# neeharperi/FutureDet

Measured on AMD Instinct MI355X. Metric: sweeps/sec end-to-end (300k pts, 10-sweep voxel), higher is better.
Workload: dtype f32

## Files before the change

### futuredet_amd/backbones.py

```python
import numpy as np
import torch
from torch import nn

from . import hip_ops, sparse as spconv
from .nn_utils import build_norm_layer
from .registry import BACKBONES
from .sparse import SparseConv3d, SubMConv3d


def conv3x3(in_planes, out_planes, stride=1, indice_key=None, bias=True):
    return spconv.SubMConv3d(in_planes, out_planes, kernel_size=3, stride=stride, padding=1, bias=bias,
                             indice_key=indice_key)


class SparseBasicBlock(spconv.SparseModule):
    expansion = 1

    def __init__(self, inplanes, planes, stride=1, norm_cfg=None, downsample=None, indice_key=None):
        super().__init__()
        if norm_cfg is None:
            norm_cfg = dict(type="BN1d", eps=1e-3, momentum=0.01)
        bias = norm_cfg is not None
        self.conv1 = conv3x3(inplanes, planes, stride, indice_key=indice_key, bias=bias)
        self.bn1 = build_norm_layer(norm_cfg, planes)[1]
        self.relu = nn.ReLU()
        self.conv2 = conv3x3(planes, planes, indice_key=indice_key, bias=bias)
        self.bn2 = build_norm_layer(norm_cfg, planes)[1]
        self.downsample = downsample
        self.stride = stride

    def forward(self, x):
        identity = x
        out = self.conv1(x)
        out.features = self.relu(self.bn1(out.features))
        out = self.conv2(out)
        out.features = self.bn2(out.features)
        if self.downsample is not None:
            identity = self.downsample(x)
        out.features = self.relu(out.features + identity.features)
        return out


@BACKBONES.register_module
class SpMiddleResNetFHD(nn.Module):
    def __init__(self, num_input_features=128, norm_cfg=None, name="SpMiddleResNetFHD", **kwargs):
        super().__init__()
        self.name = name
        if norm_cfg is None:
            norm_cfg = dict(type="BN1d", eps=1e-3, momentum=0.01)
        S = spconv.SparseSequential
        self.conv_input = S(SubMConv3d(num_input_features, 16, 3, bias=False, indice_key="res0"),
                            build_norm_layer(norm_cfg, 16)[1], nn.ReLU(inplace=True))
        self.conv1 = S(SparseBasicBlock(16, 16, norm_cfg=norm_cfg, indice_key="res0"),
                       SparseBasicBlock(16, 16, norm_cfg=norm_cfg, indice_key="res0"))
        self.conv2 = S(SparseConv3d(16, 32, 3, 2, padding=1, bias=False), build_norm_layer(norm_cfg, 32)[1],
                       nn.ReLU(inplace=True), SparseBasicBlock(32, 32, norm_cfg=norm_cfg, indice_key="res1"),
                       SparseBasicBlock(32, 32, norm_cfg=norm_cfg, indice_key="res1"))
        self.conv3 = S(SparseConv3d(32, 64, 3, 2, padding=1, bias=False), build_norm_layer(norm_cfg, 64)[1],
                       nn.ReLU(inplace=True), SparseBasicBlock(64, 64, norm_cfg=norm_cfg, indice_key="res2"),
                       SparseBasicBlock(64, 64, norm_cfg=norm_cfg, indice_key="res2"))
        self.conv4 = S(SparseConv3d(64, 128, 3, 2, padding=[0, 1, 1], bias=False), build_norm_layer(norm_cfg, 128)[1],
                       nn.ReLU(inplace=True), SparseBasicBlock(128, 128, norm_cfg=norm_cfg, indice_key="res3"),
                       SparseBasicBlock(128, 128, norm_cfg=norm_cfg, indice_key="res3"))
        self.extra_conv = S(SparseConv3d(128, 128, (3, 1, 1), (2, 1, 1), bias=False), build_norm_layer(norm_cfg, 128)[1],
                            nn.ReLU())
        self.compute_dtype = torch.float32
        self.dense_channels_last = True
        self.dense_dtype = None
        self.profile_hook = None

    def forward_generic(self, voxel_features, coors, batch_size, input_shape):
        sparse_shape = np.array(input_shape[::-1]) + [1, 0, 0]
        ret = spconv.SparseConvTensor(voxel_features, coors.int(), sparse_shape, batch_size)
        x = self.conv_input(ret)
        x_conv1 = self.conv1(x)
        x_conv2 = self.conv2(x_conv1)
        x_conv3 = self.conv3(x_conv2)
        x_conv4 = self.conv4(x_conv3)
        ret = self.extra_conv(x_conv4).dense()
        N, C, D, H, W = ret.shape
        ret = ret.view(N, C * D, H, W)
        return ret, {"conv1": x_conv1, "conv2": x_conv2, "conv3": x_conv3, "conv4": x_conv4}

    def _stages(self):
        return [(self.conv_input[0], self.conv_input[1], [self.conv1[0], self.conv1[1]], True),
                (self.conv2[0], self.conv2[1], [self.conv2[3], self.conv2[4]], False),
                (self.conv3[0], self.conv3[1], [self.conv3[3], self.conv3[4]], False),
                (self.conv4[0], self.conv4[1], [self.conv4[3], self.conv4[4]], False),
                (self.extra_conv[0], self.extra_conv[1], [], False)]

    def build_indexes(self, mark_fn, batch_size, input_shape, device, voxels=None, static=False, expected=None, row_caps=None):
        D, H, W = [int(v) for v in (np.array(input_shape[::-1]) + [1, 0, 0])]
        if voxels is not None:
            geoms = [self._stages()[lvl][0].geometry() for lvl in range(1, 5)]
            return hip_ops.build_pyramid(voxels[0], voxels[1], voxels[2], batch_size, (D, H, W), geoms, device, static=static,
                                         expected=expected, row_caps=row_caps)
        assert not static, "static indexes are built from the voxelizer's device output (voxels=...)"
        counts = torch.zeros((5,), dtype=torch.int32, device=device)
        idx = [hip_ops.SparseIndex(batch_size, D, H, W, device)]
        mark_fn(idx[0])
        idx[0].scan(counts[0:1])
        for lvl in range(1, 5):
            conv = self._stages()[lvl][0]
            ks, st, pd = conv.geometry()
            nxt = idx[-1].downsample(ks, st, pd)
            nxt.scan(counts[lvl:lvl + 1])
            idx.append(nxt)
        host = counts.cpu()
        for i, ix in enumerate(idx):
            ix.finalize(int(host[i]))
        return idx

    def run_fused(self, idx, feats0, dense_out=None, fork=False):
        dt = self.compute_dtype
        stages = self._stages()
        rb_cache = {}

        def rulebook(src, dst, conv):
            ks, st, pd = conv.geometry()
            key = (id(src), id(dst), tuple(ks), tuple(st), tuple(pd))
            if key not in rb_cache:
                rb_cache[key] = src.rulebook(dst, ks, st, pd)
            return rb_cache[key]

        def run(conv, bn, x, src, dst, relu, residual=None):
            wpk, bias, cin_p, cout_p = conv.packed_weight(dt, bn)
            assert x.shape[1] == cin_p, (x.shape, cin_p)
            nbr = rulebook(src, dst, conv)
            fn = lambda: hip_ops.spconv_apply(x, wpk, bias, nbr, dst.n, cout_p, residual=residual, relu=relu)
            if self.profile_hook is not None:
                s = 4 if dt == torch.float32 else 2
                K = nbr.shape[0]
                pairs = lambda: int((nbr[:, : dst.n] >= 0).sum().item())
                return self.profile_hook("spconv_%dx%d_K%d" % (cin_p, cout_p, K),
                                         dict(s=s, K=K, cin=cin_p, cout=cout_p, n_in=src.n, n_out=dst.n, pairs=pairs), fn)
            return fn()

        main, side = None, None
        if fork and feats0.is_cuda:
            main = torch.cuda.current_stream(feats0.device)
            pool = self.__dict__.setdefault("_side_streams", {})
            side = pool.get(main.cuda_stream)
            if side is None:
                side = pool[main.cuda_stream] = torch.cuda.Stream(device=feats0.device)
            side.wait_stream(main)
            with torch.cuda.stream(side):
                made = []
                for lvl, (conv, bn, blocks, is_subm_in) in enumerate(stages):
                    if lvl == 0:
                        continue
                    src_l, dst_l = (idx[lvl] if is_subm_in else idx[lvl - 1]), idx[lvl]
                    made.append(rulebook(src_l, dst_l, conv))
                    for blk in blocks:
                        nbr = rulebook(dst_l, dst_l, blk.conv1)
                        made.append(nbr)
                        cp = spconv.pad_channels(blk.conv1.out_channels)
                        if dt == torch.float32 and nbr.shape[0] == 27 and \
                                hip_ops._lib.load().fd_spconv_wants_balanced_ranges(cp, cp, 0):
                            r = hip_ops.ranges_for(nbr, cp, cp)
                            if r[0] is not None:
                                made.append(r[0])
                for t in made:
                    t.record_stream(main)
        x = feats0
        levels = {}
        for lvl, (conv, bn, blocks, is_subm_in) in enumerate(stages):
            src = idx[lvl] if is_subm_in else idx[lvl - 1]
            dst = idx[lvl]
            if lvl == 1 and side is not None:
                main.wait_stream(side)
            x = run(conv, bn, x, src, dst, relu=True)
            for blk in blocks:
                y = run(blk.conv1, blk.bn1, x, dst, dst, relu=True)
                x = run(blk.conv2, blk.bn2, y, dst, dst, relu=True, residual=x)
            levels[lvl] = (x, dst)
        bev = hip_ops.densify(x, idx[4], out_dtype=self.dense_dtype or dt, channels_last=self.dense_channels_last, out=dense_out)
        return bev, levels

    def forward(self, voxel_features, coors, batch_size, input_shape):
        if self.training:
            if self.compute_dtype != torch.float32 and torch.is_grad_enabled():
                raise NotImplementedError("SpMiddleResNetFHD: training runs the fp32 sparse convolution only; the %s path is inference-only "
                                          "(set compute_dtype = torch.float32 to train)" % self.compute_dtype)
            return self.forward_generic(voxel_features, coors, batch_size, input_shape)
        coors = coors.int().contiguous()
        dev = voxel_features.device
        idx = self.build_indexes(lambda i0: i0.mark(coors), batch_size, input_shape, dev)
        row_of = idx[0].lookup(coors)
        feats0 = hip_ops.rows_permute(voxel_features.float().contiguous(), row_of,
                                      spconv.pad_channels(voxel_features.shape[1]), self.compute_dtype, n_rows=idx[0].n)
        bev, levels = self.run_fused(idx, feats0)
        multi = {}
        for name, lvl, c in (("conv1", 0, 16), ("conv2", 1, 32), ("conv3", 2, 64), ("conv4", 3, 128)):
            f, ix = levels[lvl]
            multi[name] = spconv.SparseConvTensor(f[:, :c], None, ix.spatial_shape, batch_size, _index=ix)
        return bev, multi


@BACKBONES.register_module
class PointPillarsScatter(nn.Module):

    def __init__(self, num_input_features=64, norm_cfg=None, name="PointPillarsScatter", **kwargs):
        super().__init__()
        self.name = "PointPillarsScatter"
        self.nchannels = num_input_features
        self.dense_channels_last = True

    def forward(self, voxel_features, coords, batch_size, input_shape, n_dev=None):
        self.nx = int(input_shape[0])
        self.ny = int(input_shape[1])
        coords = coords.int().contiguous()
        if n_dev is None and torch.is_grad_enabled() and voxel_features.requires_grad:
            return _ScatterFn.apply(voxel_features, coords, batch_size, self.ny, self.nx, self.dense_channels_last)
        return hip_ops.pillar_scatter(voxel_features, coords, n_dev, batch_size, self.ny, self.nx,
                                      channels_last=self.dense_channels_last)


class _ScatterFn(torch.autograd.Function):

    @staticmethod
    def forward(ctx, feats, coords, batch_size, ny, nx, channels_last):
        ctx.coords = coords
        return hip_ops.pillar_scatter(feats, coords, None, batch_size, ny, nx, channels_last=channels_last)

    @staticmethod
    def backward(ctx, dcanvas):
        d = hip_ops.pillar_scatter_backward(dcanvas.float(), ctx.coords)
        ctx.coords = None
        return d, None, None, None, None, None
```

### futuredet_amd/csrc/fd_common.h

```cpp
#pragma once
#include <hip/hip_runtime.h>
#include <stdint.h>
#include <stdio.h>

#include <atomic>

#include "../../include/futuredet_hip.h"

namespace fd {

void set_error(const char *fmt, ...);
int spconv_f32_compact_dispatch(const float *in, const void *wp, const float *bias, const float *residual, int relu, const int *nbr,
                                int64_t nbr_stride, int K, int64_t n_in_bound, int n_out, const int *n_out_dev, int cin, int cout, float *out,
                                const int *ranges, int n_ranges, hipStream_t stream);

size_t spconv_bf16_win_weight_bytes(int K, int cin, int cout);
void spconv_bf16_win_pack(const float *w, int K, int cin, int cout, uint16_t (*tobf)(float), uint16_t *dst);
int spconv_bf16_win_dispatch(const void *in, const void *wp_win, const float *bias, const void *residual, int relu, const int *nbr, int64_t nbr_stride, int K,
                             int64_t n_in_bound, int n_out, const int *n_out_dev, int64_t n_expected, int cin, int cout, void *out, hipStream_t stream);
int spconv_bf16_ws_dispatch(const void *in, const void *wp, const float *bias, const void *residual, int relu, const int *nbr, int64_t nbr_stride, int K,
                            int64_t n_in_bound, int n_out, const int *n_out_dev, int64_t n_expected, int cin, int cout, void *out, hipStream_t stream);

int wino_pc_launch(const float *x, const void *wp, const float *bias, float *y, int B, int H, int W, int cin, int cout, int relu, int cout_total,
                   int co_off, int wide_items, hipStream_t stream);

int spconv_f32_res16_dispatch(const float *in, const void *wp, const float *bias, const float *residual, int relu, const int *nbr, int64_t nbr_stride, int K,
                              int64_t n_in_bound, int n_out, const int *n_out_dev, int64_t n_expected, int cin, int cout, float *out, hipStream_t stream);

int spconv_f32_c32_dispatch(const float *in, const void *wp, const float *bias, const float *residual, int relu, const int *nbr,
                            int64_t nbr_stride, int K, int64_t n_in_bound, int n_out, const int *n_out_dev, int cin, int cout, float *out,
                            const int *ranges, int n_ranges, hipStream_t stream);

__device__ __forceinline__ int device_count(int capacity, const int *count_dev) {
    if (!count_dev) return capacity;
    const int n = *count_dev;
    return n < capacity ? (n > 0 ? n : 0) : capacity;
}

inline int check_launch(const char *what) {
    hipError_t e = hipGetLastError();
    if (e != hipSuccess) {
        set_error("%s: %s", what, hipGetErrorString(e));
        return FD_ELAUNCH;
    }
    return FD_OK;
}

#define FD_REQUIRE(cond, ...)           \
    do {                                \
        if (!(cond)) {                  \
            fd::set_error(__VA_ARGS__); \
            return FD_EINVAL;           \
        }                               \
    } while (0)

inline hipStream_t as_stream(fd_stream_t s) { return reinterpret_cast<hipStream_t>(s); }

int fill_words(void *p, uint32_t value, size_t n_words, hipStream_t stream);
int fill_words3(void *p0, uint32_t v0, size_t n0, void *p1, uint32_t v1, size_t n1, void *p2, uint32_t v2, size_t n2, hipStream_t stream);

constexpr int kMaxDevices = 64;
int current_device();
int device_cu_count();
bool ensure_dynamic_lds(const void *kernel, size_t bytes, std::atomic<uint64_t> &done);
enum TuneKey { kTuneSpconvRG = 0, kTuneSpconvV1, kTuneSpconvBf16V1, kTuneV2Depth, kTuneV2TM, kTuneV2LdsPad, kTuneConvNT, kTuneV2RangesPerCU, kTuneV2Uniform, kTuneV2RowCost, kTuneSpconvC32, kTuneBf16GP, kTuneBf16RG, kTuneBf16Depth, kTuneBf16NW, kTuneStrict, kTuneBf16Win, kTuneF32ResRG, kTuneConvStrip, kTuneF32ResNW, kTuneCount };
int tuning(TuneKey key);

inline size_t align_up(size_t v, size_t a) { return (v + a - 1) / a * a; }

struct IndexGeom {
    int B, D, H, W, Ht, Wt;
    __host__ __device__ int64_t num_cols() const { return (int64_t)B * Ht * Wt * 64; }
};
__host__ __device__ inline IndexGeom make_geom(int B, int D, int H, int W) {
    IndexGeom g;
    g.B = B; g.D = D; g.H = H; g.W = W;
    g.Ht = (H + 7) >> 3; g.Wt = (W + 7) >> 3;
    return g;
}
__host__ __device__ inline int64_t col_of(const IndexGeom &g, int b, int y, int x) {
    return ((((int64_t)b * g.Ht + (y >> 3)) * g.Wt + (x >> 3)) << 6) + ((y & 7) << 3) + (x & 7);
}
__device__ inline void col_to_byx(const IndexGeom &g, int64_t col, int &b, int &y, int &x) {
    int in = (int)(col & 63);
    int64_t t = col >> 6;
    int tx = (int)(t % g.Wt);
    t /= g.Wt;
    int ty = (int)(t % g.Ht);
    b = (int)(t / g.Ht);
    y = ty * 8 + (in >> 3);
    x = tx * 8 + (in & 7);
}

__device__ inline unsigned xcd_swizzle(unsigned bid, unsigned nblocks) {
    const unsigned nx = 8;
    unsigned per = nblocks / nx, rem = nblocks % nx;
    unsigned xcd = bid % nx, loc = bid / nx;
    unsigned start = xcd * per + (xcd < rem ? xcd : rem);
    return start + loc;
}

}
```

### futuredet_amd/csrc/fd_spconv.hip

```cpp
#include "fd_common.h"

namespace {

typedef float f32x4 __attribute__((ext_vector_type(4)));
typedef short s16x4 __attribute__((ext_vector_type(4)));
typedef __bf16 bf16x8 __attribute__((ext_vector_type(8)));

__device__ inline unsigned short f2bf(float v) {
    unsigned u = __float_as_uint(v);
    u += 0x7fffu + ((u >> 16) & 1u);
    return (unsigned short)(u >> 16);
}
__device__ inline float bf2f(unsigned short h) { return __uint_as_float(((unsigned)h) << 16); }

constexpr int kMaxTaps = 27;

template <int CIN, int COUT, int RG>
__global__ void __launch_bounds__(256) spconv_f32(const float *__restrict__ in, const float4 *__restrict__ wp,
                                                  const float *__restrict__ bias, const float *__restrict__ residual, int relu,
                                                  const int *__restrict__ nbr, int64_t nbr_stride, int K, int n_out,
                                                  const int *__restrict__ n_out_dev, float *__restrict__ out) {
    constexpr int ROWS_B = 64 * RG;
    constexpr int NB = COUT / 16, NC = CIN / 16;
    __shared__ int s_nbr[kMaxTaps * ROWS_B];
    const int tile = blockIdx.x;
    const int row0 = tile * ROWS_B;
    n_out = fd::device_count(n_out, n_out_dev);
    if (row0 >= n_out) return;
    for (int t = threadIdx.x; t < K * ROWS_B; t += 256) {
        int k = t / ROWS_B, r = t - k * ROWS_B;
        int64_t o = (int64_t)row0 + r;
        s_nbr[t] = (o < n_out) ? nbr[(int64_t)k * nbr_stride + o] : -1;
    }
    __syncthreads();
    const int lane = threadIdx.x & 63, wave = __builtin_amdgcn_readfirstlane(threadIdx.x >> 6);
    const int lrow = lane & 15, lq = lane >> 4;
    const int wrow = wave * 16 * RG;
    if (row0 + wrow >= n_out) return;

    f32x4 acc[RG][NB];
#pragma unroll
    for (int g = 0; g < RG; ++g)
#pragma unroll
        for (int nb = 0; nb < NB; ++nb) acc[g][nb] = (f32x4){0.f, 0.f, 0.f, 0.f};

    for (int k = 0; k < K; ++k) {
        int idx[RG];
        bool any[RG];
        bool any_all = false;
#pragma unroll
        for (int g = 0; g < RG; ++g) {
            idx[g] = s_nbr[k * ROWS_B + wrow + g * 16 + lrow];
            any[g] = __ballot(idx[g] >= 0) != 0ull;
            any_all = any_all || any[g];
        }
        if (!any_all) continue;
        const float4 *wk = wp + (int64_t)k * NC * NB * 64 + lane;
#pragma unroll
        for (int c = 0; c < NC; ++c) {
            float4 a[RG];
#pragma unroll
            for (int g = 0; g < RG; ++g) {
                a[g] = make_float4(0.f, 0.f, 0.f, 0.f);
                if (idx[g] >= 0) a[g] = *reinterpret_cast<const float4 *>(in + (int64_t)idx[g] * CIN + c * 16 + lq * 4);
            }
#pragma unroll
            for (int nb = 0; nb < NB; ++nb) {
                const float4 b = wk[(c * NB + nb) * 64];
#pragma unroll
                for (int g = 0; g < RG; ++g) {
                    if (any[g]) {
                        acc[g][nb] = __builtin_amdgcn_mfma_f32_16x16x4f32(a[g].x, b.x, acc[g][nb], 0, 0, 0);
                        acc[g][nb] = __builtin_amdgcn_mfma_f32_16x16x4f32(a[g].y, b.y, acc[g][nb], 0, 0, 0);
                        acc[g][nb] = __builtin_amdgcn_mfma_f32_16x16x4f32(a[g].z, b.z, acc[g][nb], 0, 0, 0);
                        acc[g][nb] = __builtin_amdgcn_mfma_f32_16x16x4f32(a[g].w, b.w, acc[g][nb], 0, 0, 0);
                    }
                }
            }
        }
    }
#pragma unroll
    for (int g = 0; g < RG; ++g) {
#pragma unroll
        for (int nb = 0; nb < NB; ++nb) {
            const int col = nb * 16 + lrow;
            const float bv = bias ? bias[col] : 0.0f;
#pragma unroll
            for (int r = 0; r < 4; ++r) {
                const int row = row0 + wrow + g * 16 + lq * 4 + r;
                if (row < n_out) {
                    float v = acc[g][nb][r] + bv;
                    if (residual) v += residual[(int64_t)row * COUT + col];
                    if (relu) v = fmaxf(v, 0.0f);
                    out[(int64_t)row * COUT + col] = v;
                }
            }
        }
    }
}

template <int CIN, int COUT, int RG>
__global__ void __launch_bounds__(256) spconv_bf16(const unsigned short *__restrict__ in, const void *__restrict__ wp_,
                                                   const float *__restrict__ bias, const unsigned short *__restrict__ residual,
                                                   int relu, const int *__restrict__ nbr, int64_t nbr_stride, int K, int n_out,
                                                   const int *__restrict__ n_out_dev, unsigned short *__restrict__ out) {
    constexpr int ROWS_B = 64 * RG;
    constexpr int NB = COUT / 16;
    constexpr bool WIDE = CIN >= 32;
    constexpr int NC = WIDE ? CIN / 32 : 1;
    __shared__ int s_nbr[kMaxTaps * ROWS_B];
    const int tile = blockIdx.x;
    const int row0 = tile * ROWS_B;
    n_out = fd::device_count(n_out, n_out_dev);
    if (row0 >= n_out) return;
    for (int t = threadIdx.x; t < K * ROWS_B; t += 256) {
        int k = t / ROWS_B, r = t - k * ROWS_B;
        int64_t o = (int64_t)row0 + r;
        s_nbr[t] = (o < n_out) ? nbr[(int64_t)k * nbr_stride + o] : -1;
    }
    __syncthreads();
    const int lane = threadIdx.x & 63, wave = __builtin_amdgcn_readfirstlane(threadIdx.x >> 6);
    const int lrow = lane & 15, lq = lane >> 4;
    const int wrow = wave * 16 * RG;
    if (row0 + wrow >= n_out) return;

    f32x4 acc[RG][NB];
#pragma unroll
    for (int g = 0; g < RG; ++g)
#pragma unroll
        for (int nb = 0; nb < NB; ++nb) acc[g][nb] = (f32x4){0.f, 0.f, 0.f, 0.f};

    for (int k = 0; k < K; ++k) {
        int idx[RG];
        bool any[RG];
        bool any_all = false;
#pragma unroll
        for (int g = 0; g < RG; ++g) {
            idx[g] = s_nbr[k * ROWS_B + wrow + g * 16 + lrow];
            any[g] = __ballot(idx[g] >= 0) != 0ull;
            any_all = any_all || any[g];
        }
        if (!any_all) continue;
        if constexpr (WIDE) {
            const bf16x8 *wk = reinterpret_cast<const bf16x8 *>(wp_) + (int64_t)k * NC * NB * 64 + lane;
#pragma unroll
            for (int c = 0; c < NC; ++c) {
                bf16x8 a[RG];
#pragma unroll
                for (int g = 0; g < RG; ++g) {
                    uint4 raw = make_uint4(0u, 0u, 0u, 0u);
                    if (idx[g] >= 0) raw = *reinterpret_cast<const uint4 *>(in + (int64_t)idx[g] * CIN + c * 32 + lq * 8);
                    a[g] = __builtin_bit_cast(bf16x8, raw);
                }
#pragma unroll
                for (int nb = 0; nb < NB; ++nb) {
                    const bf16x8 b = wk[(c * NB + nb) * 64];
#pragma unroll
                    for (int g = 0; g < RG; ++g)
                        if (any[g]) acc[g][nb] = __builtin_amdgcn_mfma_f32_16x16x32_bf16(a[g], b, acc[g][nb], 0, 0, 0);
                }
            }
        } else {
            const s16x4 *wk = reinterpret_cast<const s16x4 *>(wp_) + (int64_t)k * NB * 64 + lane;
            s16x4 a[RG];
#pragma unroll
            for (int g = 0; g < RG; ++g) {
                uint2 raw = make_uint2(0u, 0u);
                if (idx[g] >= 0) raw = *reinterpret_cast<const uint2 *>(in + (int64_t)idx[g] * CIN + lq * 4);
                a[g] = __builtin_bit_cast(s16x4, raw);
            }
#pragma unroll
            for (int nb = 0; nb < NB; ++nb) {
                const s16x4 b = wk[nb * 64];
#pragma unroll
                for (int g = 0; g < RG; ++g)
                    if (any[g]) acc[g][nb] = __builtin_amdgcn_mfma_f32_16x16x16bf16_1k(a[g], b, acc[g][nb], 0, 0, 0);
            }
        }
    }
#pragma unroll
    for (int g = 0; g < RG; ++g) {
#pragma unroll
        for (int nb = 0; nb < NB; ++nb) {
            const int col = nb * 16 + lrow;
            const float bv = bias ? bias[col] : 0.0f;
#pragma unroll
            for (int r = 0; r < 4; ++r) {
                const int row = row0 + wrow + g * 16 + lq * 4 + r;
                if (row < n_out) {
                    float v = acc[g][nb][r] + bv;
                    if (residual) v += bf2f(residual[(int64_t)row * COUT + col]);
                    if (relu) v = fmaxf(v, 0.0f);
                    out[(int64_t)row * COUT + col] = f2bf(v);
                }
            }
        }
    }
}

struct LaunchArgs {
    const void *in, *wp;
    const float *bias;
    const void *residual;
    int relu;
    const int *nbr;
    int64_t nbr_stride;
    int K, n_out;
    const int *n_out_dev;
    void *out;
    hipStream_t stream;
};

template <int CIN, int COUT, int RG>
void launch(const LaunchArgs &a, int dtype) {
    const int rows_b = 64 * RG;
    dim3 grid((unsigned)((a.n_out + rows_b - 1) / rows_b));
    if (dtype == 0)
        hipLaunchKernelGGL((spconv_f32<CIN, COUT, RG>), grid, dim3(256), 0, a.stream, (const float *)a.in, (const float4 *)a.wp, a.bias,
                           (const float *)a.residual, a.relu, a.nbr, a.nbr_stride, a.K, a.n_out, a.n_out_dev, (float *)a.out);
    else
        hipLaunchKernelGGL((spconv_bf16<CIN, COUT, RG>), grid, dim3(256), 0, a.stream, (const unsigned short *)a.in, a.wp, a.bias,
                           (const unsigned short *)a.residual, a.relu, a.nbr, a.nbr_stride, a.K, a.n_out, a.n_out_dev, (unsigned short *)a.out);
}

template <int CIN, int COUT>
void launch_rg(const LaunchArgs &a, int dtype, int rg) {
    if (rg >= 4) launch<CIN, COUT, 4>(a, dtype);
    else if (rg == 2) launch<CIN, COUT, 2>(a, dtype);
    else launch<CIN, COUT, 1>(a, dtype);
}

int pick_rg(int64_t n_out, int cin, int cout) {
    const int forced = fd::tuning(fd::kTuneSpconvRG);
    if (forced > 0) return forced;
    const int64_t waves2 = (n_out + 31) / 32;
    int rg = (cin * cout >= 128 * 128) ? 1 : 2;
    if (rg == 2 && waves2 < 256 * 4 * 2) rg = 1;
    return rg;
}

}

inline bool has_c32_layout(int cin, int cout, int dtype) { return dtype == 0 && cout == 32 && cin == 32; }
inline int64_t pair_layout_elems(int K, int cin, int cout, int dtype) { return (dtype == 1 && cin == 16) ? (int64_t)((K + 1) / 2) * 32 * cout : 0; }

extern "C" size_t fd_spconv_packed_weight_bytes(int K, int cin, int cout, int dtype) {
    if (K <= 0 || cin <= 0 || cout <= 0) return 0;
    return (size_t)K * cin * cout * (dtype == 0 ? 4 : 2) * (has_c32_layout(cin, cout, dtype) ? 2 : 1) + (size_t)pair_layout_elems(K, cin, cout, dtype) * 2 +
           (dtype == 1 ? fd::spconv_bf16_win_weight_bytes(K, cin, cout) : 0);
}

extern "C" int fd_spconv_pack_weight(const float *w, int K, int cin, int cout, int dtype, void *dst) {
    FD_REQUIRE(w && dst, "fd_spconv_pack_weight: null argument");
    FD_REQUIRE(K >= 1 && K <= kMaxTaps, "fd_spconv_pack_weight: K must be in [1,27]");
    FD_REQUIRE(cin % 16 == 0 && cout % 16 == 0 && cin >= 16 && cin <= 128 && cout >= 16 && cout <= 128,
               "fd_spconv_pack_weight: channels must be multiples of 16 in [16,128] (got %d -> %d)", cin, cout);
    FD_REQUIRE(dtype == 0 || dtype == 1, "fd_spconv_pack_weight: dtype must be 0 (f32) or 1 (bf16)");
    const int NB = cout / 16;
    auto W = [&](int k, int ci, int co) { return w[((int64_t)k * cin + ci) * cout + co]; };
    auto tobf = [](float v) -> uint16_t {
        union { float f; uint32_t u; } cvt;
        cvt.f = v;
        uint32_t u = cvt.u;
        u += 0x7fffu + ((u >> 16) & 1u);
        return (uint16_t)(u >> 16);
    };
    if (dtype == 0) {
        const int NC = cin / 16;
        float *d = (float *)dst;
        for (int k = 0; k < K; ++k)
            for (int c = 0; c < NC; ++c)
                for (int nb = 0; nb < NB; ++nb)
                    for (int lane = 0; lane < 64; ++lane)
                        for (int j = 0; j < 4; ++j)
                            d[((((int64_t)k * NC + c) * NB + nb) * 64 + lane) * 4 + j] =
                                W(k, 16 * c + 4 * (lane >> 4) + j, 16 * nb + (lane & 15));
        if (has_c32_layout(cin, cout, dtype)) {
            float *e = d + (int64_t)K * cin * cout;
            for (int k = 0; k < K; ++k)
                for (int c = 0; c < cin / 8; ++c)
                    for (int lane = 0; lane < 64; ++lane)
                        for (int j = 0; j < 4; ++j)
                            e[(((int64_t)k * (cin / 8) + c) * 64 + lane) * 4 + j] = W(k, 8 * c + 4 * (lane >> 5) + j, lane & 31);
        }
    } else if (cin >= 32) {
        FD_REQUIRE(cin % 32 == 0, "fd_spconv_pack_weight: bf16 needs cin 16 or a multiple of 32");
        const int NC = cin / 32;
        uint16_t *d = (uint16_t *)dst;
        for (int k = 0; k < K; ++k)
            for (int c = 0; c < NC; ++c)
                for (int nb = 0; nb < NB; ++nb)
                    for (int lane = 0; lane < 64; ++lane)
                        for (int j = 0; j < 8; ++j)
                            d[((((int64_t)k * NC + c) * NB + nb) * 64 + lane) * 8 + j] =
                                tobf(W(k, 32 * c + 8 * (lane >> 4) + j, 16 * nb + (lane & 15)));
        if (fd::spconv_bf16_win_weight_bytes(K, cin, cout)) fd::spconv_bf16_win_pack(w, K, cin, cout, +tobf, d + (int64_t)K * cin * cout);
    } else {
        uint16_t *d = (uint16_t *)dst;
        for (int k = 0; k < K; ++k)
            for (int nb = 0; nb < NB; ++nb)
                for (int lane = 0; lane < 64; ++lane)
                    for (int j = 0; j < 4; ++j)
                        d[(((int64_t)k * NB + nb) * 64 + lane) * 4 + j] = tobf(W(k, 4 * (lane >> 4) + j, 16 * nb + (lane & 15)));
        uint16_t *e = d + (int64_t)K * cin * cout;
        for (int u = 0; u < (K + 1) / 2; ++u)
            for (int nb = 0; nb < NB; ++nb)
                for (int lane = 0; lane < 64; ++lane)
                    for (int j = 0; j < 8; ++j) {
                        const int q = lane >> 4, k = 2 * u + (q >> 1);
                        e[(((int64_t)u * NB + nb) * 64 + lane) * 8 + j] = k < K ? tobf(W(k, 8 * (q & 1) + j, 16 * nb + (lane & 15))) : (uint16_t)0;
                    }
    }
    return FD_OK;
}

extern "C" int fd_spconv_apply(const void *in_feats, int64_t n_in, const void *wpacked, const float *bias, const void *residual, int relu,
                               const int32_t *nbr, int64_t nbr_stride, const int32_t *ranges, int n_ranges, int K, int64_t n_out,
                               const int32_t *n_out_dev, int64_t n_expected, int cin, int cout, int dtype, void *out_feats, fd_stream_t stream) {
    FD_REQUIRE(K >= 1 && K <= kMaxTaps, "fd_spconv_apply: K must be in [1,27]");
    FD_REQUIRE(dtype == 0 || dtype == 1, "fd_spconv_apply: dtype must be 0 (f32) or 1 (bf16)");
    FD_REQUIRE(n_out >= 0 && n_out <= nbr_stride && n_out < (1ll << 31), "fd_spconv_apply: n_out out of range");
    FD_REQUIRE(n_ranges >= 0 && (ranges == nullptr || n_ranges >= 1), "fd_spconv_apply: ranges needs n_ranges >= 1");
    if (n_expected <= 0 || n_expected > n_out) n_expected = n_out;
    if (n_out == 0) return FD_OK;
    FD_REQUIRE(in_feats && wpacked && nbr && out_feats, "fd_spconv_apply: null argument");
    if (dtype == 0 && !fd::tuning(fd::kTuneSpconvV1) && cin == 16 && fd::tuning(fd::kTuneF32ResRG) >= 0) {
        if (fd::spconv_f32_res16_dispatch((const float *)in_feats, wpacked, bias, (const float *)residual, relu, nbr, nbr_stride, K, n_in, (int)n_out,
                                          n_out_dev, n_expected, cin, cout, (float *)out_feats, fd::as_stream(stream)))
            return fd::check_launch("fd_spconv_apply(f32 resident)");
    }
    if (dtype == 0 && !fd::tuning(fd::kTuneSpconvV1) && has_c32_layout(cin, cout, dtype) && fd::tuning(fd::kTuneSpconvC32) >= 0) {
        const void *w32 = (const char *)wpacked + (size_t)K * cin * cout * 4;
        if (fd::spconv_f32_c32_dispatch((const float *)in_feats, w32, bias, (const float *)residual, relu, nbr, nbr_stride, K, n_in, (int)n_out,
                                        n_out_dev, cin, cout, (float *)out_feats, ranges, n_ranges, fd::as_stream(stream)))
            return fd::check_launch("fd_spconv_apply(c32)");
    }
    if (dtype == 0 && !fd::tuning(fd::kTuneSpconvV1)) {
        if (fd::spconv_f32_compact_dispatch((const float *)in_feats, wpacked, bias, (const float *)residual, relu, nbr, nbr_stride, K, n_in,
                                            (int)n_out, n_out_dev, cin, cout, (float *)out_feats, ranges, n_ranges, fd::as_stream(stream)))
            return fd::check_launch("fd_spconv_apply(compact)");
    }
    if (dtype == 1 && fd::tuning(fd::kTuneBf16GP) >= 0) {
        const void *w = cin == 16 ? (const void *)((const char *)wpacked + (size_t)K * cin * cout * 2) : wpacked;
        const bool subm_like = (K == 27 && n_in == n_out) || fd::tuning(fd::kTuneBf16Win) == 2;
        if (fd::tuning(fd::kTuneBf16Win) >= 0 && subm_like && fd::spconv_bf16_win_weight_bytes(K, cin, cout) &&
            fd::spconv_bf16_win_dispatch(in_feats, (const char *)wpacked + (size_t)K * cin * cout * 2, bias, residual, relu, nbr, nbr_stride, K, n_in, (int)n_out,
                                         n_out_dev, n_expected, cin, cout, out_feats, fd::as_stream(stream)))
            return fd::check_launch("fd_spconv_apply(bf16 window)");
        if (fd::spconv_bf16_ws_dispatch(in_feats, w, bias, residual, relu, nbr, nbr_stride, K, n_in, (int)n_out, n_out_dev, n_expected, cin, cout, out_feats,
                                        fd::as_stream(stream)))
            return fd::check_launch("fd_spconv_apply(bf16 ws)");
        if (fd::tuning(fd::kTuneStrict) && n_in * cin * 2 < (1ll << 31)) {
            fd::set_error("fd_spconv_apply: strict mode: the bf16 kernel (fd_spconv_bf16.hip) did not take %d -> %d, K = %d", cin, cout, K);
            return FD_EINVAL;
        }
    }
    LaunchArgs a{in_feats, wpacked, bias, residual, relu, nbr, nbr_stride, K, (int)n_out, n_out_dev, out_feats, fd::as_stream(stream)};
    const int rg = pick_rg(n_expected, cin, cout);
    const int key = cin * 1000 + cout;
    switch (key) {
        case 16016: launch_rg<16, 16>(a, dtype, rg); break;
        case 16032: launch_rg<16, 32>(a, dtype, rg); break;
        case 32032: launch_rg<32, 32>(a, dtype, rg); break;
        case 32064: launch_rg<32, 64>(a, dtype, rg); break;
        case 64064: launch_rg<64, 64>(a, dtype, rg); break;
        case 64128: launch_rg<64, 128>(a, dtype, rg); break;
        case 128128: launch_rg<128, 128>(a, dtype, rg); break;
        default:
            fd::set_error("fd_spconv_apply: unsupported channels %d -> %d", cin, cout);
            return FD_EINVAL;
    }
    return fd::check_launch("fd_spconv_apply");
}
```

### futuredet_amd/csrc/fd_spconv_c32.hip

```cpp
#include "fd_spconv_chunk.h"

namespace {

namespace sk = fd::skeleton;
typedef float f32x16 __attribute__((ext_vector_type(16)));
typedef unsigned u32x4 __attribute__((ext_vector_type(4)));
constexpr int TM = 128, COUT = 32, TS = 4, WR = 1;
constexpr sk::Layout L = sk::layout(TM, COUT, TS, 32);
static_assert(((sk::kMaxTaps + TS - 1) / TS) * (TM / WR / 32) <= L.item_slot, "item list slot");

template <int CIN, int DEPTH>
__global__ void __launch_bounds__(256) spconv_f32_c32(const float *__restrict__ in, const float4 *__restrict__ wp, const float *__restrict__ bias,
                                                      const float *__restrict__ residual, int relu, const int *__restrict__ nbr, int64_t nbr_stride,
                                                      int K, int n_out, const int *__restrict__ n_out_dev, float *__restrict__ out, unsigned in_bytes,
                                                      const int *__restrict__ ranges, int rows_per_range) {
    constexpr int NCH = CIN / 8;
    constexpr int kPad = sk::pad_entry(TM);
    extern __shared__ __attribute__((aligned(16))) unsigned char smem[];
    int *s_list = reinterpret_cast<int *>(smem + L.list);
    unsigned short *s_items = reinterpret_cast<unsigned short *>(smem + L.items);
    unsigned char *s_cnt = smem + L.cnt;
    int *s_pad = reinterpret_cast<int *>(smem + L.pad);
    float *s_acc = reinterpret_cast<float *>(smem + L.acc);

    const int tid = threadIdx.x, lane = tid & 63, wave = __builtin_amdgcn_readfirstlane(tid >> 6);
    int r_begin, r_end, n_chunks, chunk_rows;
    sk::resolve_range(n_out, n_out_dev, ranges, rows_per_range, r_begin, r_end);
    if (r_begin >= r_end) return;
    sk::cut_chunks<TM>(r_begin, r_end, n_chunks, chunk_rows);
    int pre[sk::kSliceRegs<TM>];
    sk::fetch_slice<TM>(pre, nbr, nbr_stride, K, r_begin);

    const int ln = lane & 31, lh = lane >> 5;
    const int ts = wave, wr = 0;
    unsigned char *acc_bytes = reinterpret_cast<unsigned char *>(s_acc + ts * L.acc_copy);
    const __amdgpu_buffer_rsrc_t rsrc = __builtin_amdgcn_make_buffer_rsrc(const_cast<float *>(in), 0, (int)in_bytes, 0x00020000);
    unsigned short *items = s_items + wave * L.item_slot;

    for (int chunk = 0; chunk < n_chunks; ++chunk) {
        int row0, n_rows;
        if (!sk::chunk_span(r_begin, r_end, chunk_rows, chunk, row0, n_rows)) break;
        sk::stage_chunk<TM, COUT, TS, 32>(pre, s_list, s_pad, s_acc, bias, residual, K, row0, n_rows);
        __syncthreads();
        sk::compact_taps<TM, WR>(s_list, s_cnt, K);
        __syncthreads();
        if (chunk + 1 < n_chunks) sk::fetch_slice<TM>(pre, nbr, nbr_stride, K, row0 + chunk_rows);
        const int n_items = sk::build_items<TS, 32>(s_cnt, items, K, ts, wr);

        int k_r[DEPTH], row_r[DEPTH];
        u32x4 a_r[DEPTH][NCH];
        auto stage_a0 = [&](int it) -> int { return sk::stage_a0(items, n_items, it); };
        auto stage_a1 = [&](int it, int code_v, int &kk, int &e) { sk::stage_a1<TM, WR, 32>(s_list, s_pad, n_items, wr, ln, it, code_v, kk, e); };
        auto gather_offset = [&](int e) -> unsigned { return sk::entry_row_bytes<CIN>(e) + (unsigned)(lh * 16); };
        auto gather_step = [&](unsigned voff, int c) { return __builtin_amdgcn_raw_buffer_load_b128(rsrc, voff + c * 32, 0, 0); };
        float4 b[NCH];
        auto load_b = [&](int k) {
            const float4 *wk = wp + (int64_t)k * NCH * 64 + lane;
#pragma unroll
            for (int c = 0; c < NCH; ++c) b[c] = wk[c * 64];
        };
        int k_s, e_s, code_s;
#pragma unroll
        for (int d = 0; d < DEPTH - 1; ++d) {
            stage_a1(d, stage_a0(d), k_s, e_s);
            const unsigned vo = gather_offset(e_s);
#pragma unroll
            for (int c = 0; c < NCH; ++c) a_r[d][c] = gather_step(vo, c);
            k_r[d] = k_s;
            row_r[d] = e_s;
        }
        k_r[DEPTH - 1] = -1;
        row_r[DEPTH - 1] = kPad;
        stage_a1(DEPTH - 1, stage_a0(DEPTH - 1), k_s, e_s);
        code_s = stage_a0(DEPTH);
        if (n_items > 0) load_b(k_r[0]);

        for (int i0 = 0; i0 < n_items; i0 += DEPTH) {
#pragma unroll
            for (int d = 0; d < DEPTH; ++d) {
                const unsigned arow = sk::entry_local_row(row_r[d]);
                unsigned aoff[4];
#pragma unroll
                for (int q = 0; q < 4; ++q) aoff[q] = sk::acc_slot_bytes<COUT>(arow, (unsigned)(2 * q + lh));
                f32x16 acc;
#pragma unroll
                for (int q = 0; q < 4; ++q) {
                    const float4 v = *reinterpret_cast<const float4 *>(acc_bytes + aoff[q]);
                    acc[4 * q + 0] = v.x; acc[4 * q + 1] = v.y; acc[4 * q + 2] = v.z; acc[4 * q + 3] = v.w;
                }
                const int dn = (d + DEPTH - 1) % DEPTH;
                {
                    const int it = i0 + d + DEPTH - 1;
                    const unsigned vo = gather_offset(e_s);
                    k_r[dn] = k_s;
                    row_r[dn] = e_s;
#pragma unroll
                    for (int c = 0; c < NCH; ++c) a_r[dn][c] = gather_step(vo, c);
                    stage_a1(it + 1, code_s, k_s, e_s);
                    code_s = stage_a0(it + 2);
                }
                const int knext = k_r[(d + 1) % DEPTH];
                const bool reload = knext >= 0 && knext != k_r[d];
                __builtin_amdgcn_sched_barrier(0);
#pragma unroll
                for (int c = 0; c < NCH; ++c) {
                    const float4 av = __builtin_bit_cast(float4, a_r[d][c]);
                    acc = __builtin_amdgcn_mfma_f32_32x32x2f32(b[c].x, av.x, acc, 0, 0, 0);
                    acc = __builtin_amdgcn_mfma_f32_32x32x2f32(b[c].y, av.y, acc, 0, 0, 0);
                    acc = __builtin_amdgcn_mfma_f32_32x32x2f32(b[c].z, av.z, acc, 0, 0, 0);
                    acc = __builtin_amdgcn_mfma_f32_32x32x2f32(b[c].w, av.w, acc, 0, 0, 0);
                    if (reload) b[c] = (wp + (int64_t)knext * NCH * 64 + lane)[c * 64];
                }
#pragma unroll
                for (int q = 0; q < 4; ++q)
                    *reinterpret_cast<float4 *>(acc_bytes + aoff[q]) = make_float4(acc[4 * q + 0], acc[4 * q + 1], acc[4 * q + 2], acc[4 * q + 3]);
                __builtin_amdgcn_sched_barrier(0);
            }
        }
        __syncthreads();
        sk::epilogue<TM, COUT, TS>(s_acc, bias, residual, relu, out, row0, n_rows);
        __syncthreads();
    }
}

template <int CIN, int DEPTH>
int launch_c32(const float *in, const void *wp, const float *bias, const float *residual, int relu, const int *nbr, int64_t nbr_stride, int K,
               int n_out, const int *n_out_dev, float *out, unsigned in_bytes, const int *ranges, int n_ranges, hipStream_t stream) {
    int rows_per = 0;
    if (!ranges) sk::equal_rows_split(n_out, TM, n_out_dev != nullptr, n_ranges, rows_per);
    static std::atomic<uint64_t> lds_set{0};
    if (!fd::ensure_dynamic_lds(reinterpret_cast<const void *>(spconv_f32_c32<CIN, DEPTH>), (size_t)L.bytes, lds_set)) return 0;
    hipLaunchKernelGGL((spconv_f32_c32<CIN, DEPTH>), dim3((unsigned)n_ranges), dim3(256), (size_t)L.bytes, stream, in, (const float4 *)wp, bias, residual, relu,
                       nbr, nbr_stride, K, n_out, n_out_dev, out, in_bytes, ranges, rows_per);
    return 1;
}

}

namespace fd {
int spconv_f32_c32_dispatch(const float *in, const void *wp, const float *bias, const float *residual, int relu, const int *nbr, int64_t nbr_stride,
                            int K, int64_t n_in_bound, int n_out, const int *n_out_dev, int cin, int cout, float *out, const int *ranges,
                            int n_ranges, hipStream_t stream) {
    if (cout != 32 || cin != 32) return 0;
    if (!sk::entries_fit(n_in_bound, cin)) return 0;
    const unsigned in_bytes = (unsigned)(n_in_bound * cin * 4);
    const int depth = fd::tuning(fd::kTuneV2Depth);
    if (depth == 2) return launch_c32<32, 2>(in, wp, bias, residual, relu, nbr, nbr_stride, K, n_out, n_out_dev, out, in_bytes, ranges, n_ranges, stream);
    if (depth == 4) return launch_c32<32, 4>(in, wp, bias, residual, relu, nbr, nbr_stride, K, n_out, n_out_dev, out, in_bytes, ranges, n_ranges, stream);
    return launch_c32<32, 3>(in, wp, bias, residual, relu, nbr, nbr_stride, K, n_out, n_out_dev, out, in_bytes, ranges, n_ranges, stream);
}
}
```

### futuredet_amd/csrc/fd_spconv_chunk.h

```cpp
#pragma once
#include "fd_common.h"

namespace fd {
namespace skeleton {

constexpr int kMaxTaps = 27;

constexpr int pad_entry(int tm) { return (int)(0xffffff00u | (unsigned)tm); }
__device__ __forceinline__ int pack_entry(int in_row, int local_row) { return (in_row << 8) | local_row; }
__device__ __forceinline__ unsigned entry_local_row(int e) { return (unsigned)e & 255u; }
template <int CIN>
__device__ __forceinline__ unsigned entry_row_bytes(int e) {
    static_assert(CIN == 16 || CIN == 32 || CIN == 64 || CIN == 128, "shift per CIN");
    const unsigned hi = (unsigned)e & 0xffffff00u;
    return CIN >= 64 ? hi << (CIN == 128 ? 1 : 0) : hi >> (CIN == 32 ? 1 : 2);
}
inline bool entries_fit(int64_t n_in_bound, int cin) { return n_in_bound < (1ll << 23) && n_in_bound * cin * 4 < (1ll << 31); }

struct Layout {
    int list;
    int items;
    int item_slot;
    int cnt;
    int pad;
    int acc;
    int acc_copy;
    int bytes;
};
constexpr int acc_copy_floats(int tm, int cout) { return (tm + 1) * cout; }
constexpr Layout layout(int tm, int cout, int ts, int item) {
    Layout l{};
    l.list = 0;
    l.items = l.list + (int)sizeof(int) * kMaxTaps * tm;
    l.item_slot = item == 16 ? kMaxTaps * (tm / 16) : 32;
    l.cnt = l.items + (int)sizeof(unsigned short) * 4 * l.item_slot;
    l.pad = l.cnt + 112;
    l.acc = l.pad + (int)sizeof(int) * item;
    l.acc_copy = acc_copy_floats(tm, cout);
    l.bytes = l.acc + (int)sizeof(float) * ts * l.acc_copy;
    return l;
}

template <int COUT>
__device__ __forceinline__ unsigned acc_swizzle(unsigned row) {
    static_assert(COUT == 16 || COUT == 32 || COUT == 64 || COUT == 128, "whole bank rows");
    constexpr int kSwzShift = COUT >= 64 ? 0 : COUT == 32 ? 1 : 2;
    constexpr unsigned kSwzMask = COUT >= 64 ? 15u : COUT == 32 ? 7u : 3u;
    return (row >> kSwzShift) & kSwzMask;
}
template <int COUT>
__device__ __forceinline__ int acc_slot(int row, int col) {
    return row * (COUT / 4) + (col ^ (int)acc_swizzle<COUT>((unsigned)row));
}
template <int COUT>
__device__ __forceinline__ unsigned acc_slot_bytes(unsigned row, unsigned col) {
    return row * (COUT * 4) + ((col ^ acc_swizzle<COUT>(row)) << 4);
}

__device__ __forceinline__ void resolve_range(int n_out, const int *n_out_dev, const int *ranges, int rows_per_range,
                                              int &r_begin, int &r_end) {
    if (n_out_dev) n_out = fd::device_count(n_out, n_out_dev);
    if (ranges) {
        r_begin = ranges[blockIdx.x];
        r_end = ranges[blockIdx.x + 1];
    } else {
        if (n_out_dev) rows_per_range = (((n_out + (int)gridDim.x - 1) / (int)gridDim.x) + 15) & ~15;
        const int64_t b = (int64_t)blockIdx.x * rows_per_range;
        r_begin = (int)(b < n_out ? b : n_out);
        r_end = (int)(b + rows_per_range < n_out ? b + rows_per_range : n_out);
    }
    if (r_end > n_out) r_end = n_out;
}
template <int TM>
__device__ __forceinline__ void cut_chunks(int r_begin, int r_end, int &n_chunks, int &chunk_rows) {
    n_chunks = (r_end - r_begin + TM - 1) / TM;
    chunk_rows = (((r_end - r_begin + n_chunks - 1) / n_chunks) + 15) & ~15;
}
__device__ __forceinline__ bool chunk_span(int r_begin, int r_end, int chunk_rows, int chunk, int &row0, int &n_rows) {
    row0 = r_begin + chunk * chunk_rows;
    n_rows = (r_end - row0) < chunk_rows ? (r_end - row0) : chunk_rows;
    return n_rows > 0;
}
inline void equal_rows_split(int n_out, int tm, bool device_count, int &n_ranges, int &rows_per) {
    if (n_ranges <= 0) n_ranges = (n_out + tm - 1) / tm;
    rows_per = (((n_out + n_ranges - 1) / n_ranges) + 15) & ~15;
    if (!device_count) n_ranges = (n_out + rows_per - 1) / rows_per;
}

template <int TM>
constexpr int kSliceRegs = (kMaxTaps * TM + 255) / 256;

template <int TM>
__device__ __forceinline__ void fetch_slice(int (&pre)[kSliceRegs<TM>], const int *nbr, int64_t nbr_stride, int K, int row0) {
    const int tid = threadIdx.x;
#pragma unroll
    for (int i = 0; i < kSliceRegs<TM>; ++i) {
        const int t = tid + i * 256;
        int k = t / TM;
        const int r = t - k * TM;
        k = k < K ? k : K - 1;
        int64_t o = (int64_t)row0 + r;
        o = o < nbr_stride ? o : nbr_stride - 1;
        pre[i] = nbr[(int64_t)k * nbr_stride + o];
    }
}

template <int COUT>
constexpr bool kInitAcc = COUT <= 64;

template <int TM, int COUT, int TS>
__device__ __forceinline__ void init_acc(float *s_acc, const float *bias, const float *residual, int row0, int n_rows) {
    const int tid = threadIdx.x;
    if constexpr (kInitAcc<COUT>) {
        constexpr int C4i = COUT / 4, NINIT = TM * C4i / 256;
        static_assert(TM * C4i % 256 == 0, "whole passes");
        float4 iv[NINIT];
#pragma unroll
        for (int i = 0; i < NINIT; ++i) {
            const int t = tid + i * 256, c4 = t % C4i;
            iv[i] = bias ? reinterpret_cast<const float4 *>(bias)[c4] : make_float4(0.f, 0.f, 0.f, 0.f);
        }
        if (residual) {
            float4 rv[NINIT];
#pragma unroll
            for (int i = 0; i < NINIT; ++i) {
                const int t = tid + i * 256, r = t / C4i, c4 = t - r * C4i;
                const int rr = r < n_rows ? r : n_rows - 1;
                rv[i] = reinterpret_cast<const float4 *>(residual + (int64_t)(row0 + rr) * COUT)[c4];
            }
#pragma unroll
            for (int i = 0; i < NINIT; ++i) { iv[i].x += rv[i].x; iv[i].y += rv[i].y; iv[i].z += rv[i].z; iv[i].w += rv[i].w; }
        }
#pragma unroll
        for (int i = 0; i < NINIT; ++i) {
            const int t = tid + i * 256, r = t / C4i, c4 = t - r * C4i;
            reinterpret_cast<float4 *>(s_acc)[acc_slot<COUT>(r, c4)] = r < n_rows ? iv[i] : make_float4(0.f, 0.f, 0.f, 0.f);
        }
        for (int t = TM * C4i + tid; t < TS * acc_copy_floats(TM, COUT) / 4; t += 256) reinterpret_cast<float4 *>(s_acc)[t] = make_float4(0.f, 0.f, 0.f, 0.f);
    } else {
        for (int t = tid; t < TS * acc_copy_floats(TM, COUT) / 4; t += 256) reinterpret_cast<float4 *>(s_acc)[t] = make_float4(0.f, 0.f, 0.f, 0.f);
    }
}

template <int TM, int COUT, int TS, int ITEM>
__device__ __forceinline__ void stage_chunk(const int (&pre)[kSliceRegs<TM>], int *s_list, int *s_pad, float *s_acc, const float *bias,
                                            const float *residual, int K, int row0, int n_rows) {
    const int tid = threadIdx.x;
    static_assert(256 % TM == 0, "a thread stages the same local row in every pass");
    const bool in_chunk = tid % TM < n_rows;
#pragma unroll
    for (int i = 0; i < kSliceRegs<TM>; ++i) {
        const int t = tid + i * 256;
        if (t < K * TM) s_list[t] = in_chunk ? pre[i] : -1;
    }
    init_acc<TM, COUT, TS>(s_acc, bias, residual, row0, n_rows);
    if (tid < ITEM) s_pad[tid] = pad_entry(TM);
}

template <int TM, int WR>
__device__ __forceinline__ void compact_taps(int *s_list, unsigned char *s_cnt, int K) {
    const int lane = threadIdx.x & 63, wave = __builtin_amdgcn_readfirstlane(threadIdx.x >> 6);
    constexpr int RW = TM / WR, NH = (RW + 63) / 64;
    for (int k = wave; k < K; k += 4) {
#pragma unroll
        for (int wr = 0; wr < WR; ++wr) {
            const int base = k * TM + wr * RW;
            int count = 0;
            int v[NH];
#pragma unroll
            for (int h = 0; h < NH; ++h) {
                const int r = h * 64 + lane;
                v[h] = (r < RW) ? s_list[base + r] : -1;
            }
#pragma unroll
            for (int h = 0; h < NH; ++h) {
                const int r = h * 64 + lane;
                if (r < RW) s_list[base + r] = pad_entry(TM);
            }
#pragma unroll
            for (int h = 0; h < NH; ++h) {
                const int r = h * 64 + lane;
                const unsigned long long m = __ballot(v[h] >= 0);
                const int pos = count + __popcll(m & ((1ull << lane) - 1ull));
                if (v[h] >= 0) s_list[base + pos] = pack_entry(v[h], wr * RW + r);
                count += __popcll(m);
            }
            if (lane == 0) s_cnt[k * 4 + wr] = (unsigned char)count;
        }
    }
}

template <int TS, int ITEM>
__device__ __forceinline__ int build_items(const unsigned char *s_cnt, unsigned short *items, int K, int ts, int wr) {
    const int lane = threadIdx.x & 63;
    const int ng = (lane < K && (lane % TS) == ts) ? ((int)s_cnt[lane * 4 + wr] + ITEM - 1) / ITEM : 0;
    int inc = ng;
#pragma unroll
    for (int off = 1; off < 64; off <<= 1) {
        const int u = __shfl_up(inc, off);
        if (lane >= off) inc += u;
    }
    const int n_items = __builtin_amdgcn_readfirstlane(__shfl(inc, 63));
    for (int g = 0; g < ng; ++g) items[inc - ng + g] = (unsigned short)((lane << 3) | g);
    __builtin_amdgcn_fence(__ATOMIC_RELEASE, "workgroup");
    __builtin_amdgcn_wave_barrier();
    __builtin_amdgcn_fence(__ATOMIC_ACQUIRE, "workgroup");
    return n_items;
}

__device__ __forceinline__ int stage_a0(const unsigned short *items, int n_items, int it) { return (int)items[it < n_items ? it : 0]; }
template <int TM, int WR, int ITEM>
__device__ __forceinline__ void stage_a1(const int *s_list, const int *s_pad, int n_items, int wr, int lp, int it, int code_v, int &kk, int &e) {
    const bool v = it < n_items;
    const int code = __builtin_amdgcn_readfirstlane(code_v);
    const int ks = v ? (code >> 3) : 0;
    kk = v ? ks : -1;
    const int *lst = v ? s_list + ks * TM + wr * (TM / WR) + (code & 7) * ITEM : s_pad;
    e = lst[lp];
}

template <int TM, int COUT, int TS>
__device__ __forceinline__ void epilogue(float *s_acc, const float *bias, const float *residual, int relu,
                                         float *out, int row0, int n_rows) {
    const int tid = threadIdx.x;
    constexpr int C4 = COUT / 4;
    for (int t = tid; t < n_rows * C4; t += 256) {
        const int r = t / C4, c4 = t - r * C4;
        const int row = row0 + r;
        const int slot = acc_slot<COUT>(r, c4);
        float4 v = reinterpret_cast<const float4 *>(s_acc)[slot];
#pragma unroll
        for (int q = 1; q < TS; ++q) {
            const float4 v2 = reinterpret_cast<const float4 *>(s_acc + q * acc_copy_floats(TM, COUT))[slot];
            v.x += v2.x; v.y += v2.y; v.z += v2.z; v.w += v2.w;
        }
        if constexpr (!kInitAcc<COUT>) {
            if (bias) {
                const float4 bv = reinterpret_cast<const float4 *>(bias)[c4];
                v.x += bv.x; v.y += bv.y; v.z += bv.z; v.w += bv.w;
            }
            if (residual) {
                const float4 rv = reinterpret_cast<const float4 *>(residual + (int64_t)row * COUT)[c4];
                v.x += rv.x; v.y += rv.y; v.z += rv.z; v.w += rv.w;
            }
        }
        if (relu) { v.x = fmaxf(v.x, 0.f); v.y = fmaxf(v.y, 0.f); v.z = fmaxf(v.z, 0.f); v.w = fmaxf(v.w, 0.f); }
        reinterpret_cast<float4 *>(out + (int64_t)row * COUT)[c4] = v;
    }
}

}
}
```

### futuredet_amd/hip_ops.py

```python
import ctypes
import threading

import numpy as np
import torch

from . import lib as _lib
from .lib import DecodeCfg, FutureDetHipError, MapView, check


_raw_stream = getattr(torch._C, "_cuda_getCurrentRawStream", None)


def _stream():
    if _raw_stream is not None:
        return ctypes.c_void_p(_raw_stream(torch.cuda.current_device()))
    return ctypes.c_void_p(torch.cuda.current_stream().cuda_stream)


def _dev(t, name, dtype=None):
    if not isinstance(t, torch.Tensor) or not t.is_cuda:
        raise FutureDetHipError("%s must be a tensor on the HIP device (got %s); this path has no CPU implementation"
                                % (name, "cpu tensor" if isinstance(t, torch.Tensor) else type(t)))
    if dtype is not None and t.dtype != dtype:
        raise FutureDetHipError("%s must be %s, got %s" % (name, dtype, t.dtype))
    if not t.is_contiguous():
        raise FutureDetHipError("%s must be contiguous" % name)
    return t


def _p(t):
    return ctypes.c_void_p(t.data_ptr()) if t is not None else None


class _Workspace(object):

    def __init__(self):
        self._bufs = {}
        self._scope = threading.local()

    def scope(self, token):
        ws = self

        class _Scope(object):
            def __enter__(self_):
                self_.prev = getattr(ws._scope, "token", None)
                ws._scope.token = token

            def __exit__(self_, *exc):
                ws._scope.token = self_.prev

        return _Scope()

    def release(self, token):
        for key in [k for k in self._bufs if k[2] == ("scope", token)]:
            del self._bufs[key]

    def get(self, tag, nbytes, device):
        token = getattr(self._scope, "token", None)
        key = (tag, device.index, ("scope", token) if token is not None else _stream().value)
        buf = self._bufs.get(key)
        if buf is None or buf.numel() < nbytes:
            buf = torch.empty(max(int(nbytes), 256), dtype=torch.uint8, device=device)
            self._bufs[key] = buf
        return buf


workspace = _Workspace()
_DT = {torch.float32: 0, torch.bfloat16: 1}


def set_tuning(name, value):
    check(_lib.load().fd_tuning_set(name.encode(), int(value)), "fd_tuning_set")


def voxelize(points, voxel_size, coors_range, max_points, max_voxels, batch_idx=0, want_voxels=True, want_mean=False,
             mean_stride=None, coor_cols=3, out=None, n_points_dev=None):
    L = _lib.load()
    points = _dev(points, "points", torch.float32)
    n, ndim = points.shape
    dev = points.device
    rng = (ctypes.c_float * 6)(*[float(np.float32(v)) for v in coors_range])
    vs = (ctypes.c_float * 3)(*[float(np.float32(v)) for v in voxel_size])
    out = dict(out or {})
    if want_voxels and "voxels" not in out:
        out["voxels"] = torch.empty((max_voxels, max_points, ndim), dtype=torch.float32, device=dev)
    if want_mean and "mean" not in out:
        out["mean"] = torch.empty((max_voxels, mean_stride or ndim), dtype=torch.float32, device=dev)
    if "coors" not in out:
        out["coors"] = torch.empty((max_voxels, coor_cols), dtype=torch.int32, device=dev)
    if "num_points" not in out:
        out["num_points"] = torch.empty((max_voxels,), dtype=torch.int32, device=dev)
    if "num_voxels" not in out:
        out["num_voxels"] = torch.zeros((1,), dtype=torch.int32, device=dev)
    mean = out.get("mean") if want_mean else None
    voxels = out.get("voxels") if want_voxels else None
    ws_bytes = L.fd_voxelize_workspace_bytes(n, max_voxels)
    ws = workspace.get("voxelize", ws_bytes, dev)
    check(L.fd_voxelize(_p(points), n, _p(n_points_dev), ndim, rng, vs, int(max_points), int(max_voxels), int(batch_idx), _p(voxels), _p(mean),
                        int(mean.shape[1]) if mean is not None else 0, _p(out["coors"]), int(out["coors"].shape[1]),
                        _p(out["num_points"]), _p(out["num_voxels"]), _p(ws), ws.numel(), _stream()), "fd_voxelize")
    return out


class SparseIndex(object):

    def __init__(self, B, D, H, W, device, words=None, prefix=None):
        L = _lib.load()
        self.B, self.D, self.H, self.W = int(B), int(D), int(H), int(W)
        self.ncols = L.fd_index_num_cols(self.B, self.H, self.W)
        self.words = torch.zeros((self.ncols,), dtype=torch.int64, device=device) if words is None else words
        self.prefix = torch.empty((self.ncols,), dtype=torch.int32, device=device) if prefix is None else prefix
        self.n_dev = None
        self.n = None
        self.coords = None
        self.device = device
        self.static = False
        self.n_expected = 0

    @property
    def spatial_shape(self):
        return [self.D, self.H, self.W]

    def mark(self, coords, n_dev=None, n_max=None):
        L = _lib.load()
        coords = _dev(coords, "coords", torch.int32)
        n_max = coords.shape[0] if n_max is None else n_max
        check(L.fd_index_mark(_p(coords), _p(n_dev), n_max, self.B, self.D, self.H, self.W, _p(self.words), _stream()),
              "fd_index_mark")

    def scan(self, n_dev):
        L = _lib.load()
        ws = workspace.get("index_scan", L.fd_index_workspace_bytes(self.ncols), self.device)
        self.n_dev = n_dev
        check(L.fd_index_scan(_p(self.words), self.ncols, _p(self.prefix), _p(n_dev), _p(ws), ws.numel(), _stream()),
              "fd_index_scan")

    def downsample(self, ksize, stride, pad):
        L = _lib.load()
        od = [(i + 2 * p - (k - 1) - 1) // s + 1 for i, k, s, p in zip(self.spatial_shape, ksize, stride, pad)]
        out = SparseIndex(self.B, od[0], od[1], od[2], self.device)
        check(L.fd_index_downsample(_p(self.words), self.B, self.D, self.H, self.W, (ctypes.c_int * 3)(*ksize),
                                    (ctypes.c_int * 3)(*stride), (ctypes.c_int * 3)(*pad), _p(out.words), _stream()),
              "fd_index_downsample")
        return out

    def finalize(self, n):
        L = _lib.load()
        self.n = int(n)
        self.coords = torch.empty((max(self.n, 1), 4), dtype=torch.int32, device=self.device)[: self.n]
        if self.n:
            check(L.fd_index_coords(_p(self.words), _p(self.prefix), self.B, self.D, self.H, self.W, _p(self.coords),
                                    _stream()), "fd_index_coords")

    def lookup(self, coords, n_dev=None):
        L = _lib.load()
        coords = _dev(coords, "coords", torch.int32)
        row_of = torch.empty((coords.shape[0],), dtype=torch.int32, device=self.device)
        check(L.fd_index_lookup(_p(self.words), _p(self.prefix), self.B, self.D, self.H, self.W, _p(coords), _p(n_dev),
                                coords.shape[0], _p(row_of), _stream()), "fd_index_lookup")
        return row_of

    def rulebook(self, out_index, ksize, stride, pad):
        L = _lib.load()
        assert out_index.n is not None
        K = int(ksize[0] * ksize[1] * ksize[2])
        nstride = max(64, (out_index.n + 63) // 64 * 64)
        nbr = torch.empty((K, nstride), dtype=torch.int32, device=self.device)
        static = getattr(out_index, "static", False)
        if out_index.n == 0:
            nbr.fill_(-1)
            return nbr
        check(L.fd_rulebook(_p(self.words), _p(self.prefix), self.B, self.D, self.H, self.W, _p(out_index.coords), out_index.n,
                            _p(out_index.n_dev), nstride, 0 if static else 1, (ctypes.c_int * 3)(*ksize), (ctypes.c_int * 3)(*stride),
                            (ctypes.c_int * 3)(*pad), _p(nbr), _stream()), "fd_rulebook")
        nbr.n_out = out_index.n
        nbr.n_dev = out_index.n_dev if static else None
        nbr.n_expected = out_index.n_expected if static else 0
        return nbr


class _PyramidPlan(object):

    def __init__(self, B, shape0, geoms, device):
        L = _lib.load()
        self.B, self.geoms, self.device = int(B), geoms, device
        self.shapes = [tuple(int(v) for v in shape0)]
        for ks, st, pd in geoms:
            self.shapes.append(tuple((i + 2 * p - (k - 1) - 1) // s + 1 for i, k, s, p in zip(self.shapes[-1], ks, st, pd)))
        self.ncols = [L.fd_index_num_cols(self.B, sh[1], sh[2]) for sh in self.shapes]
        self.ws_bytes = L.fd_index_workspace_bytes(sum(self.ncols) + 2048 * len(self.ncols))

    def row_caps(self, cap0):
        caps = [min(int(cap0), self.B * int(np.prod(self.shapes[0])))]
        for (ks, st, pd), sh in zip(self.geoms, self.shapes[1:]):
            fan = int(np.prod([-(-k // s) for k, s in zip(ks, st)]))
            caps.append(min(caps[-1] * fan, self.B * int(np.prod(sh))))
        return caps


_pyramid_plans = {}


def build_pyramid(coors, nvox, n_max, B, shape0, geoms, device, static=False, expected=None, row_caps=None):
    L = _lib.load()
    key = (int(B), tuple(int(v) for v in shape0), tuple((tuple(k), tuple(s), tuple(p)) for k, s, p in geoms), str(device))
    plan = _pyramid_plans.get(key)
    if plan is None:
        plan = _pyramid_plans[key] = _PyramidPlan(B, shape0, geoms, device)
    shapes, ncols = plan.shapes, plan.ncols
    words_all = torch.empty((sum(ncols),), dtype=torch.int64, device=device)
    prefix_all = torch.empty((sum(ncols),), dtype=torch.int32, device=device)
    counts = torch.empty((len(shapes),), dtype=torch.int32, device=device)
    idx, off = [], 0
    levels = (_lib.IndexLevel * len(shapes))()
    wp, pp = words_all.data_ptr(), prefix_all.data_ptr()
    for l, (sh, nc) in enumerate(zip(shapes, ncols)):
        ix = SparseIndex.__new__(SparseIndex)
        ix.B, ix.D, ix.H, ix.W, ix.ncols, ix.device = plan.B, sh[0], sh[1], sh[2], nc, device
        ix.words, ix.prefix = words_all[off:off + nc], prefix_all[off:off + nc]
        ix.n_dev, ix.n, ix.coords = counts[l:l + 1], None, None
        ix.level_counts = counts
        ix.static, ix.n_expected = False, 0
        lv = levels[l]
        lv.D, lv.H, lv.W = sh
        if l:
            ks, st, pd = geoms[l - 1]
            lv.ksize[:], lv.stride[:], lv.pad[:] = list(ks), list(st), list(pd)
        lv.words, lv.prefix, lv.coords = wp + 8 * off, pp + 4 * off, None
        idx.append(ix)
        off += nc
    ws = workspace.get("index_scan", plan.ws_bytes, device)

    def size_coords(host):
        total = sum(host)
        coords_all = torch.empty((max(total, 1), 4), dtype=torch.int32, device=device)
        o = 0
        for l, ix in enumerate(idx):
            ix.n = int(host[l])
            ix.coords = coords_all[o:o + ix.n]
            levels[l].coords = (coords_all.data_ptr() + 16 * o) if ix.n else None
            levels[l].coords_rows = ix.n
            o += ix.n

    if static:
        host = plan.row_caps(int(B) * int(n_max))
        if row_caps is not None:
            host = [min(int(a), int(b)) for a, b in zip(host, row_caps)]
        for l, ix in enumerate(idx):
            ix.static = True
            ix.n_expected = int(expected[l]) if expected is not None else 0
        size_coords(host)
        fused = all(int(h) > 0 for h in host)
        check(L.fd_index_pyramid(_p(coors), _p(nvox), int(n_max), plan.B, len(shapes), levels, _p(counts), _p(ws), ws.numel(), _stream()),
              "fd_index_pyramid")
        if not fused:
            check(L.fd_index_pyramid_coords(plan.B, len(shapes), levels, _stream()), "fd_index_pyramid_coords")
        return idx
    check(L.fd_index_pyramid(_p(coors), _p(nvox), int(n_max), plan.B, len(shapes), levels, _p(counts), _p(ws), ws.numel(), _stream()),
          "fd_index_pyramid")
    size_coords(counts.tolist())
    check(L.fd_index_pyramid_coords(plan.B, len(shapes), levels, _stream()), "fd_index_pyramid_coords")
    return idx


def ranges_for(nbr, cin, cout):
    cached = getattr(nbr, "ranges", None)
    if cached is not None:
        return cached
    L = _lib.load()
    n_out = getattr(nbr, "n_out", None)
    if not n_out:
        return None, 0
    K, nstride = nbr.shape
    n = int(L.fd_spconv_num_ranges(getattr(nbr, "n_expected", 0) or n_out, cin, cout, 0))
    if n <= 0:
        return None, 0
    ranges = torch.empty((n + 1,), dtype=torch.int32, device=nbr.device)
    ws = workspace.get("spconv_ranges", L.fd_spconv_ranges_workspace_bytes(n_out), nbr.device)
    check(L.fd_spconv_ranges(_p(nbr), nstride, K, n_out, _p(getattr(nbr, "n_dev", None)), n, _p(ranges), _p(ws), ws.numel(), _stream()),
          "fd_spconv_ranges")
    nbr.ranges = (ranges, n)
    return nbr.ranges


def rows_permute(src, row_of, c_dst, dtype=torch.float32, n_rows=None, n_dev=None):
    L = _lib.load()
    src = _dev(src, "src", torch.float32)
    row_of = _dev(row_of, "row_of", torch.int32)
    n_rows = src.shape[0] if n_rows is None else n_rows
    dst = torch.zeros((max(n_rows, 1), c_dst), dtype=dtype, device=src.device)[:n_rows]
    if src.shape[0]:
        check(L.fd_rows_permute(_p(src), src.shape[1], _p(row_of), _p(n_dev), src.shape[0], _p(dst), c_dst,
                                _DT[dtype], _stream()), "fd_rows_permute")
    return dst


def rows_place(index, coords, src, c_dst, dtype=torch.float32, n_dev=None, out=None):
    L = _lib.load()
    coords = _dev(coords, "coords", torch.int32)
    src = _dev(src, "src", torch.float32)
    if out is None:
        out = torch.zeros((max(index.n, 1), c_dst), dtype=dtype, device=src.device)[: index.n]
    _dev(out, "out", dtype)
    if coords.dim() != 2 or coords.shape[1] != 4:
        raise FutureDetHipError("rows_place: coords must be [n, 4] (b, z, y, x), got %s" % (tuple(coords.shape),))
    if src.dim() != 2 or src.shape[0] < coords.shape[0]:
        raise FutureDetHipError("rows_place: src must be [n, c_src] with a row per coordinate")
    if out.dim() != 2 or out.shape[1] != c_dst or index.n is None or out.shape[0] < index.n:
        raise FutureDetHipError("rows_place: out must be [rows >= index.n, %d] (finalised index), got %s" % (c_dst, tuple(out.shape)))
    check(L.fd_rows_place(_p(index.words), _p(index.prefix), index.B, index.D, index.H, index.W, _p(coords), _p(n_dev),
                          coords.shape[0], _p(src), src.shape[1], _p(out), c_dst, _DT[dtype], _stream()), "fd_rows_place")
    return out


def pack_spconv_weight(w_kio, dtype=torch.float32):
    L = _lib.load()
    dev = w_kio.device
    w = w_kio.detach().to("cpu", torch.float32).contiguous()
    K, cin, cout = w.shape
    nbytes = L.fd_spconv_packed_weight_bytes(K, cin, cout, _DT[dtype])
    host = torch.empty((nbytes,), dtype=torch.uint8)
    check(L.fd_spconv_pack_weight(ctypes.c_void_p(w.data_ptr()), K, cin, cout, _DT[dtype], ctypes.c_void_p(host.data_ptr())),
          "fd_spconv_pack_weight")
    return host.to(dev)


PACK_PLAIN, PACK_TRANSPOSED, PACK_FLIPPED_TRANSPOSED = 0, 1, 2


def pack_spconv_weight_device(w_kio, mode=PACK_PLAIN):
    L = _lib.load()
    w = _dev(w_kio.detach(), "w_kio", torch.float32)
    K, cin, cout = w.shape
    ci, co = (cout, cin) if mode else (cin, cout)
    out = torch.empty((L.fd_spconv_packed_weight_bytes(K, ci, co, 0),), dtype=torch.uint8, device=w.device)
    check(L.fd_spconv_pack_weight_device(_p(w), K, cin, cout, int(mode), _p(out), _stream()), "fd_spconv_pack_weight_device")
    return out


def spconv_wgrad(feats, dy, nbr, n_out):
    L = _lib.load()
    feats = _dev(feats, "feats", torch.float32)
    dy = _dev(dy, "dy", torch.float32)
    K, nstride = nbr.shape
    cin, cout = feats.shape[1], dy.shape[1]
    assert dy.shape[0] >= n_out
    dw = torch.empty((K, cin, cout), dtype=torch.float32, device=feats.device)
    ws = workspace.get("spconv_wgrad", L.fd_spconv_wgrad_workspace_bytes(K, n_out, cin, cout), feats.device)
    check(L.fd_spconv_wgrad(_p(feats), feats.shape[0], _p(dy), _p(_dev(nbr, "nbr", torch.int32)), nstride, K, n_out,
                            _p(getattr(nbr, "n_dev", None)), cin, cout, _p(dw), _p(ws), ws.numel(), _stream()), "fd_spconv_wgrad")
    return dw


def assign_targets(boxes, counts, classes, trajectory, cfg, out):
    L = _lib.load()
    boxes = _dev(boxes, "boxes", torch.float32)
    B = boxes.shape[0]
    assert tuple(boxes.shape) == (B, cfg.T, cfg.n_max, 12), (tuple(boxes.shape), cfg.T, cfg.n_max)
    assert tuple(counts.shape) == (B, cfg.T) and tuple(classes.shape) == (B, cfg.T, cfg.n_max)
    assert (trajectory is None) == (cfg.n_sets == 1)
    if trajectory is not None:
        assert tuple(trajectory.shape) == (B, cfg.T, cfg.n_max)
        trajectory = _dev(trajectory, "trajectory", torch.int32)
    U = cfg.n_tasks + (2 if cfg.n_sets == 3 else 0)
    ws = workspace.get("targets", L.fd_targets_workspace_bytes(B, cfg.T, U, cfg.max_objs), boxes.device)
    check(L.fd_assign_targets(_p(boxes), _p(_dev(counts, "counts", torch.int32)), _p(_dev(classes, "classes", torch.int32)), _p(trajectory), B,
                              ctypes.byref(cfg), _p(_dev(out["hm"], "hm", torch.float32)), _p(_dev(out["ind"], "ind", torch.int64)),
                              _p(_dev(out["mask"], "mask", torch.uint8)), _p(_dev(out["cat"], "cat", torch.int64)),
                              _p(_dev(out["anno_box"], "anno_box", torch.float32)), _p(_dev(out["gt_boxes_and_cls"], "gt_boxes_and_cls", torch.float32)),
                              _p(_dev(out["status"], "status", torch.int32)), _p(ws), ws.numel(), _stream()), "fd_assign_targets")
    return out


def rulebook_transpose(nbr, n_out, n_in):
    L = _lib.load()
    K, nstride = nbr.shape
    istride = max(64, (n_in + 63) // 64 * 64)
    inv = torch.empty((K, istride), dtype=torch.int32, device=nbr.device)
    check(L.fd_rulebook_transpose(_p(_dev(nbr, "nbr", torch.int32)), nstride, K, n_out, _p(getattr(nbr, "n_dev", None)), n_in, _p(inv),
                                  istride, _stream()), "fd_rulebook_transpose")
    return inv


def dense_gather(grad, index, c):
    L = _lib.load()
    if not (isinstance(grad, torch.Tensor) and grad.is_cuda and grad.dtype == torch.float32):
        raise FutureDetHipError("dense_gather: grad must be a float32 tensor on the HIP device")
    n = int(index.n)
    feats = torch.empty((max(n, 1), c), dtype=torch.float32, device=grad.device)[:n]
    sb, sc, sy, sx = grad.stride()
    check(L.fd_dense_gather(_p(grad), sb, sc, sy, sx, index.D, _p(index.coords), n, _p(index.n_dev if index.static else None), c,
                            _p(feats), _stream()), "fd_dense_gather")
    return feats


def spconv_apply(feats, wpacked, bias, nbr, n_out, cout, residual=None, relu=False, out=None, balanced=None):
    L = _lib.load()
    feats = _dev(feats, "feats")
    dt = _DT[feats.dtype]
    cin = feats.shape[1]
    out_dtype, out_cols = feats.dtype, cout
    K, nstride = nbr.shape
    if out is None:
        out = torch.empty((max(n_out, 1), out_cols), dtype=out_dtype, device=feats.device)[:n_out]
    if residual is not None:
        _dev(residual, "residual", out_dtype)
    ranges, n_ranges = None, 0
    n_dev, n_expected = getattr(nbr, "n_dev", None), getattr(nbr, "n_expected", 0)
    if dt == 0 and n_out > 0:
        if balanced is None:
            balanced = K == 27 and cin == cout and bool(L.fd_spconv_wants_balanced_ranges(cin, cout, 0))
        if balanced == "tiles":
            n_ranges = 0
        elif balanced:
            ranges, n_ranges = ranges_for(nbr, cin, cout)
        else:
            n_ranges = int(L.fd_spconv_num_ranges(n_expected or n_out, cin, cout, 0))
    check(L.fd_spconv_apply(_p(feats), feats.shape[0], _p(_dev(wpacked, "wpacked")), _p(bias), _p(residual), int(bool(relu)),
                            _p(_dev(nbr, "nbr", torch.int32)), nstride, _p(ranges), n_ranges, K, n_out, _p(n_dev), int(n_expected or 0),
                            cin, cout, dt, _p(out), _stream()),
          "fd_spconv_apply")
    return out


def densify(feats, index, out_dtype=None, channels_last=False, out=None):
    L = _lib.load()
    feats = _dev(feats, "feats")
    C = feats.shape[1]
    shape = (index.B, C * index.D, index.H, index.W)
    if out is None:
        out_dtype = out_dtype or feats.dtype
        out = torch.empty(shape, dtype=out_dtype, device=feats.device,
                          memory_format=torch.channels_last if channels_last else torch.contiguous_format)
    else:
        assert tuple(out.shape) == shape and out.is_cuda
        out_dtype = out.dtype
    sb, sc, sy, sx = out.stride()
    check(L.fd_densify(_p(feats), C, _DT[feats.dtype], _p(index.words), _p(index.prefix), index.B, index.D, index.H,
                       index.W, _p(out), _DT[out_dtype], sb, sc, sy, sx, int(feats.shape[0]), _stream()), "fd_densify")
    return out


def pack_conv2d_weight(w_oihw):
    L = _lib.load()
    dev = w_oihw.device
    w = w_oihw.detach().to("cpu", torch.float32).contiguous()
    cout, cin, ks, _ = w.shape
    nbytes = L.fd_conv2d_packed_weight_bytes(cout, cin, ks)
    if nbytes == 0:
        raise FutureDetHipError("fd_conv2d: unsupported weight shape %s" % (tuple(w.shape),))
    host = torch.empty((nbytes,), dtype=torch.uint8)
    check(L.fd_conv2d_pack_weight(ctypes.c_void_p(w.data_ptr()), cout, cin, ks, ctypes.c_void_p(host.data_ptr())),
          "fd_conv2d_pack_weight")
    return host.to(dev)


def conv2d_nhwc_bf16(x, wpk, bias, cout, ks, stride=1, relu=True, out=None, co_off=0, osy=1, osx=1, ooy=0, oox=0):
    L = _lib.load()
    x = _dev(x, "x", torch.bfloat16)
    B, H, W, cin = x.shape
    pad = 1 if ks == 3 else 0
    Ho, Wo = (H + 2 * pad - ks) // stride + 1, (W + 2 * pad - ks) // stride + 1
    if out is None:
        out = torch.empty((B, Ho * osy, Wo * osx, cout), dtype=torch.bfloat16, device=x.device)
    _dev(out, "out", torch.bfloat16)
    check(L.fd_conv2d_nhwc_bf16(_p(x), B, H, W, cin, _p(wpk), _p(bias), cout, ks, stride, pad, int(bool(relu)), _p(out),
                                out.shape[3], co_off, osy, osx, ooy, oox, _stream()), "fd_conv2d_nhwc_bf16")
    return out


def pack_conv2d_weight_f32(w_oihw):
    L = _lib.load()
    dev = w_oihw.device
    w = w_oihw.detach().to("cpu", torch.float32).contiguous()
    cout, cin, ks, _ = w.shape
    nbytes = L.fd_conv2d_f32_packed_weight_bytes(cout, cin, ks)
    if nbytes == 0:
        raise FutureDetHipError("fd_conv2d_f32: unsupported weight shape %s" % (tuple(w.shape),))
    host = torch.empty((nbytes,), dtype=torch.uint8)
    check(L.fd_conv2d_f32_pack_weight(ctypes.c_void_p(w.data_ptr()), cout, cin, ks, ctypes.c_void_p(host.data_ptr())),
          "fd_conv2d_f32_pack_weight")
    return host.to(dev)


def conv2d_nhwc_f32(x, wpk, bias, cout, ks, stride=1, relu=True, out=None, co_off=0, osy=1, osx=1, ooy=0, oox=0, tile=0):
    L = _lib.load()
    x = _dev(x, "x", torch.float32)
    B, H, W, cin = x.shape
    pad = 1 if ks == 3 else 0
    Ho, Wo = (H + 2 * pad - ks) // stride + 1, (W + 2 * pad - ks) // stride + 1
    if out is None:
        out = torch.empty((B, Ho * osy, Wo * osx, cout), dtype=torch.float32, device=x.device)
    _dev(out, "out", torch.float32)
    check(L.fd_conv2d_nhwc_f32(_p(x), B, H, W, cin, _p(wpk), _p(bias), cout, ks, stride, pad, int(bool(relu)), _p(out),
                               out.shape[3], co_off, osy, osx, ooy, oox, int(tile), _stream()), "fd_conv2d_nhwc_f32")
    return out


def conv2d_f32_num_tiles():
    return int(_lib.load().fd_conv2d_f32_num_tiles())


def conv2d_shuffle_nhwc_f32(x, wpk, bias, cout_sub, k, relu=True, out=None, co_off=0, tile=0):
    L = _lib.load()
    x = _dev(x, "x", torch.float32)
    B, H, W, cin = x.shape
    if out is None:
        out = torch.empty((B, H * k, W * k, cout_sub), dtype=torch.float32, device=x.device)
    _dev(out, "out", torch.float32)
    check(L.fd_conv2d_shuffle_nhwc_f32(_p(x), B, H, W, cin, _p(wpk), _p(bias), int(cout_sub), int(k), int(bool(relu)), _p(out), out.shape[3],
                                       co_off, int(tile), _stream()), "fd_conv2d_shuffle_nhwc_f32")
    return out


def conv2d_grouped_nhwc_f32(x, wpk, bias, counts, cin_g, relu=False, out=None, co_off=0, tile=0):
    L = _lib.load()
    x = _dev(x, "x", torch.float32)
    B, H, W, cin = x.shape
    groups = len(counts)
    assert cin == groups * cin_g
    if out is None:
        out = torch.empty((B, H, W, int(sum(counts))), dtype=torch.float32, device=x.device)
    _dev(out, "out", torch.float32)
    check(L.fd_conv2d_grouped_nhwc_f32(_p(x), B, H, W, groups, int(cin_g), _p(wpk), _p(bias), (ctypes.c_int * groups)(*[int(c) for c in counts]),
                                       int(bool(relu)), _p(out), out.shape[3], co_off, int(tile), _stream()), "fd_conv2d_grouped_nhwc_f32")
    return out


def pack_conv2d_weight_wino(w_oihw):
    L = _lib.load()
    dev = w_oihw.device
    w = w_oihw.detach().to("cpu", torch.float32).contiguous()
    cout, cin, ks, _ = w.shape
    nbytes = L.fd_conv2d_wino_f32_packed_weight_bytes(cout, cin) if ks == 3 else 0
    if nbytes == 0:
        raise FutureDetHipError("fd_conv2d_wino_f32: unsupported weight shape %s" % (tuple(w.shape),))
    host = torch.empty((nbytes,), dtype=torch.uint8)
    check(L.fd_conv2d_wino_f32_pack_weight(ctypes.c_void_p(w.data_ptr()), cout, cin, ctypes.c_void_p(host.data_ptr())),
          "fd_conv2d_wino_f32_pack_weight")
    return host.to(dev)


def conv2d_wino_nhwc_f32(x, wpk, bias, cout, relu=True, out=None, co_off=0, tile=0):
    L = _lib.load()
    x = _dev(x, "x", torch.float32)
    B, H, W, cin = x.shape
    if out is None:
        out = torch.empty((B, H, W, cout), dtype=torch.float32, device=x.device)
    _dev(out, "out", torch.float32)
    check(L.fd_conv2d_wino_nhwc_f32(_p(x), B, H, W, cin, _p(wpk), _p(bias), cout, int(bool(relu)), _p(out), out.shape[3], co_off, int(tile),
                                    _stream()), "fd_conv2d_wino_nhwc_f32")
    return out


def conv2d_wino_f32_num_tiles():
    return int(_lib.load().fd_conv2d_wino_f32_num_tiles())


CIRCLE_PRE_MAX = 4096


def pack_deform_adapt(w_cls, w_reg, off_w_cls, off_b_cls, off_w_reg, off_b_reg, bf16):
    L = _lib.load()
    dev = w_cls.device
    wc = w_cls.detach().to("cpu", torch.float32).contiguous()
    wr = w_reg.detach().to("cpu", torch.float32).contiguous()
    if tuple(wc.shape) != (64, 64, 3, 3) or tuple(wr.shape) != (64, 64, 3, 3):
        raise FutureDetHipError("fd_deform_adapt: conv_adaption weights must be [64, 64, 3, 3], got %s / %s" % (tuple(wc.shape), tuple(wr.shape)))
    host = torch.empty((L.fd_deform_adapt_packed_weight_bytes(int(bool(bf16))),), dtype=torch.uint8)
    check(L.fd_deform_adapt_pack_weight(ctypes.c_void_p(wc.data_ptr()), ctypes.c_void_p(wr.data_ptr()), int(bool(bf16)),
                                        ctypes.c_void_p(host.data_ptr())), "fd_deform_adapt_pack_weight")
    ow = torch.stack([off_w_cls.detach().float().reshape(72, 64), off_w_reg.detach().float().reshape(72, 64)]).contiguous()
    ob = torch.stack([off_b_cls.detach().float().reshape(72), off_b_reg.detach().float().reshape(72)]).contiguous()
    return host.to(dev), ow.to(dev), ob.to(dev)


def deform_adapt_nhwc(x, wpk, off_w=None, off_b=None, offsets=None, out=None):
    L = _lib.load()
    if x.dtype not in (torch.float32, torch.bfloat16):
        raise FutureDetHipError("x must be float32 or bfloat16, got %s" % (x.dtype,))
    x = _dev(x, "x")
    B, H, W, C = x.shape
    bf16 = int(x.dtype == torch.bfloat16)
    if offsets is not None:
        _dev(offsets, "offsets", torch.float32)
        if tuple(offsets.shape) != (B, H, W, 144):
            raise FutureDetHipError("offsets must be [B, H, W, 144], got %s" % (tuple(offsets.shape),))
    else:
        if off_w is None or off_b is None:
            raise FutureDetHipError("deform_adapt_nhwc: off_w and off_b are required without offsets")
        _dev(off_w, "off_w", torch.float32)
        _dev(off_b, "off_b", torch.float32)
        if off_w.numel() != 2 * 72 * C or off_b.numel() != 2 * 72:
            raise FutureDetHipError("off_w must be [2, 72, %d] and off_b [2, 72]" % C)
    if wpk.numel() != L.fd_deform_adapt_packed_weight_bytes(bf16):
        raise FutureDetHipError("deform_adapt_nhwc: packed weights are not of this dtype")
    _dev(wpk, "wpk")
    if out is None:
        out = torch.empty((B, H, W, 2 * C), dtype=x.dtype, device=x.device)
    _dev(out, "out", x.dtype)
    if tuple(out.shape) != (B, H, W, 2 * C):
        raise FutureDetHipError("out must be [B, H, W, %d], got %s" % (2 * C, tuple(out.shape)))
    check(L.fd_deform_adapt_nhwc(_p(x), B, H, W, C, bf16, _p(off_w), _p(off_b), _p(offsets), _p(wpk), _p(out), _stream()),
          "fd_deform_adapt_nhwc")
    return out


def _adapt_weight(w, name):
    w = _dev(w.detach(), name, torch.float32)
    if tuple(w.shape) != (64, 64, 3, 3):
        raise FutureDetHipError("fd_deform_adapt: %s must be [64, 64, 3, 3], got %s" % (name, tuple(w.shape)))
    return w


def pack_deform_adapt_device(w_cls, w_reg):
    L = _lib.load()
    wc, wr = _adapt_weight(w_cls, "w_cls"), _adapt_weight(w_reg, "w_reg")
    out = torch.empty((L.fd_deform_adapt_packed_weight_bytes(0),), dtype=torch.uint8, device=wc.device)
    check(L.fd_deform_adapt_pack_weight_device(_p(wc), _p(wr), _p(out), _stream()), "fd_deform_adapt_pack_weight_device")
    return out


def deform_adapt_backward(x, offsets, w_cls, w_reg, y, dy, need=(True, True, True)):
    L = _lib.load()
    x = _dev(x, "x", torch.float32)
    B, H, W, C = x.shape
    for t, name, ch in ((offsets, "offsets", 144), (y, "y", 2 * C), (dy, "dy", 2 * C)):
        _dev(t, name, torch.float32)
        if tuple(t.shape) != (B, H, W, ch):
            raise FutureDetHipError("%s must be [B, H, W, %d], got %s" % (name, ch, tuple(t.shape)))
    wc, wr = _adapt_weight(w_cls, "w_cls"), _adapt_weight(w_reg, "w_reg")
    dx = torch.empty_like(x) if need[0] else None
    doff = torch.empty_like(offsets) if need[1] else None
    dw = torch.empty((2, 64, 64, 3, 3), dtype=torch.float32, device=x.device) if need[2] else None
    ws = workspace.get("deform_adapt_backward", L.fd_deform_adapt_backward_workspace_bytes(B, H, W), x.device)
    check(L.fd_deform_adapt_backward(_p(x), _p(offsets), _p(wc), _p(wr), _p(y), _p(dy), B, H, W, C, _p(dx), _p(doff), _p(dw), _p(ws), ws.numel(),
                                     _stream()), "fd_deform_adapt_backward")
    return dx, doff, dw


def make_decode_cfg(H, W, test_cfg, hm_channels=1, group_radius=None):
    c = DecodeCfg()
    c.hm_channels = int(hm_channels)
    c.H, c.W = int(H), int(W)
    c.out_size_factor = float(test_cfg["out_size_factor"])
    c.voxel_x, c.voxel_y = float(test_cfg["voxel_size"][0]), float(test_cfg["voxel_size"][1])
    c.pc_x, c.pc_y = float(test_cfg["pc_range"][0]), float(test_cfg["pc_range"][1])
    c.score_threshold = float(test_cfg["score_threshold"])
    for i, v in enumerate(test_cfg["post_center_limit_range"]):
        c.center_range[i] = float(v)
    nms = test_cfg["nms"]
    c.nms_iou_threshold = float(nms["nms_iou_threshold"])
    c.nms_pre_max = int(nms["nms_pre_max_size"])
    c.nms_post_max = int(nms["nms_post_max_size"])
    if group_radius is not None:
        if not 1 <= len(group_radius) <= 16:
            raise ValueError("circular NMS: 1..16 decode groups, got %d radii" % len(group_radius))
        c.nms_kind, c.n_radius = 1, len(group_radius)
        c.nms_pre_max = CIRCLE_PRE_MAX
        for i, r in enumerate(group_radius):
            c.circle_radius[i] = float(r)
    return c


def centerpoint_decode(hm, reg, height, dim, rot, cfg):
    L = _lib.load()
    G = hm.shape[0]
    ts = [_dev(t, n, torch.float32) for t, n in ((hm, "hm"), (reg, "reg"), (height, "height"), (dim, "dim"), (rot, "rot"))]
    dev = hm.device
    post = cfg.nms_post_max
    boxes = torch.empty((G, post, 7), dtype=torch.float32, device=dev)
    scores = torch.empty((G, post), dtype=torch.float32, device=dev)
    cell = torch.empty((G, post), dtype=torch.int32, device=dev)
    count = torch.empty((G,), dtype=torch.int32, device=dev)
    ws = workspace.get("decode", L.fd_decode_workspace_bytes(G, ctypes.byref(cfg)), dev)
    args = []
    for t in ts:
        args += [_p(t), t.stride(0)]
    check(L.fd_centerpoint_decode(*args, G, ctypes.byref(cfg), _p(boxes), _p(scores), _p(cell), _p(count), _p(ws),
                                  ws.numel(), _stream()), "fd_centerpoint_decode")
    return boxes, scores, cell, count


def nhwc_channel_view(buf, c0):
    assert buf.is_cuda and buf.is_contiguous() and buf.dim() == 4 and buf.dtype in (torch.float32, torch.bfloat16)
    G, H, W, C = buf.shape
    return MapView(buf.data_ptr() + int(c0) * buf.element_size(), H * W * C, 1, C, 0 if buf.dtype == torch.float32 else 1)


def centerpoint_decode_views(views, G, cfg, device):
    L = _lib.load()
    post = cfg.nms_post_max
    boxes = torch.empty((G, post, 7), dtype=torch.float32, device=device)
    scores = torch.empty((G, post), dtype=torch.float32, device=device)
    cell = torch.empty((G, post), dtype=torch.int32, device=device)
    count = torch.empty((G,), dtype=torch.int32, device=device)
    ws = workspace.get("decode", L.fd_decode_workspace_bytes(G, ctypes.byref(cfg)), device)
    check(L.fd_centerpoint_decode_maps(*[ctypes.byref(v) for v in views], G, ctypes.byref(cfg), _p(boxes), _p(scores), _p(cell), _p(count), _p(ws),
                                       ws.numel(), _stream()), "fd_centerpoint_decode_maps")
    return boxes, scores, cell, count


def centerpoint_decode_packed(views, vel_view, G, B, cfg, device, step_group, step_vel_channel, step_label):
    L = _lib.load()
    post, S = cfg.nms_post_max, len(step_group)
    boxes = torch.empty((G, post, 7), dtype=torch.float32, device=device)
    scores = torch.empty((G, post), dtype=torch.float32, device=device)
    cell = torch.empty((G, post), dtype=torch.int32, device=device)
    count = torch.empty((G,), dtype=torch.int32, device=device)
    packed = torch.empty((B, S, post, 11), dtype=torch.float32, device=device)
    counts = torch.empty((B, S), dtype=torch.int32, device=device)
    ws = workspace.get("decode", L.fd_decode_workspace_bytes(G, ctypes.byref(cfg)), device)
    arr = lambda v: (ctypes.c_int32 * S)(*[int(x) for x in v])
    check(L.fd_centerpoint_decode_packed(*[ctypes.byref(v) for v in views], ctypes.byref(vel_view), int(G), int(B), ctypes.byref(cfg), S, arr(step_group),
                                         arr(step_vel_channel), arr(step_label), _p(boxes), _p(scores), _p(cell), _p(count), _p(packed), _p(counts), _p(ws),
                                         ws.numel(), _stream()), "fd_centerpoint_decode_packed")
    return packed, counts


def assemble_detections(boxes7, scores, cell, count, vel_view, B, post, step_group, step_vel_channel, step_label):
    L = _lib.load()
    S = len(step_group)
    dev = boxes7.device
    packed = torch.empty((B, S, post, 11), dtype=torch.float32, device=dev)
    counts = torch.empty((B, S), dtype=torch.int32, device=dev)
    arr = lambda v: (ctypes.c_int32 * S)(*[int(x) for x in v])
    check(L.fd_assemble_detections(_p(boxes7), _p(scores), _p(cell), _p(count), ctypes.byref(vel_view), int(B), int(post), S, arr(step_group),
                                   arr(step_vel_channel), arr(step_label), _p(packed), _p(counts), _stream()), "fd_assemble_detections")
    return packed, counts


def rotated_nms(boxes7, thresh):
    L = _lib.load()
    boxes7 = _dev(boxes7, "boxes", torch.float32)
    n = boxes7.shape[0]
    keep = torch.zeros((max(n, 1),), dtype=torch.int64, device=boxes7.device)
    count = torch.zeros((1,), dtype=torch.int32, device=boxes7.device)
    ws = workspace.get("nms", L.fd_nms_workspace_bytes(n), boxes7.device)
    check(L.fd_rotated_nms(_p(boxes7), n, ctypes.c_float(thresh), _p(keep), _p(count), _p(ws), ws.numel(), _stream()),
          "fd_rotated_nms")
    return keep, count


def boxes_iou_bev(a, b):
    L = _lib.load()
    a = _dev(a, "boxes_a", torch.float32)
    b = _dev(b, "boxes_b", torch.float32)
    out = torch.zeros((a.shape[0], b.shape[0]), dtype=torch.float32, device=a.device)
    check(L.fd_boxes_iou_bev(_p(a), a.shape[0], _p(b), b.shape[0], _p(out), _stream()), "fd_boxes_iou_bev")
    return out


SWEEP_DESC = np.dtype([("m", np.float64, (16,)), ("row_begin", np.int64), ("row_end", np.int64), ("time", np.float32),
                       ("flags", np.int32)])
SWEEP_HAS_TRANSFORM, SWEEP_REMOVE_CLOSE = 1, 2


def sweep_descriptors(rows, transforms, time_lags, remove_close):
    S = len(rows) - 1
    d = np.zeros((S,), SWEEP_DESC)
    for s in range(S):
        d["row_begin"][s], d["row_end"][s] = int(rows[s]), int(rows[s + 1])
        flags = 0
        if transforms[s] is not None:
            d["m"][s] = np.asarray(transforms[s], np.float64).reshape(16)
            flags |= SWEEP_HAS_TRANSFORM
        if remove_close[s]:
            flags |= SWEEP_REMOVE_CLOSE
        d["flags"][s] = flags
        d["time"][s] = np.float32(np.float64(time_lags[s]))
    return d


def assemble_sweeps(raw, desc, keep_cols=4, min_distance=1.0, out=None, count=None, n_sweeps=None):
    L = _lib.load()
    raw = _dev(raw, "raw", torch.float32)
    R, raw_cols = raw.shape
    dev = raw.device
    if isinstance(desc, torch.Tensor):
        desc_dev = _dev(desc, "desc", torch.uint8)
        n_desc = int(n_sweeps) if n_sweeps is not None else desc_dev.numel() // SWEEP_DESC.itemsize
        assert desc_dev.numel() >= n_desc * SWEEP_DESC.itemsize
    else:
        desc = np.ascontiguousarray(desc)
        assert desc.dtype == SWEEP_DESC
        desc_dev = torch.from_numpy(desc.view(np.uint8).reshape(-1).copy()).to(dev, non_blocking=True)
        n_desc = len(desc)
    if out is None:
        out = torch.empty((R, keep_cols + 1), dtype=torch.float32, device=dev)
    else:
        out = _dev(out, "out", torch.float32)
        assert out.shape[0] >= R and out.shape[1] == keep_cols + 1
    if count is None:
        count = torch.empty((1,), dtype=torch.int32, device=dev)
    ws_bytes = L.fd_sweep_assemble_workspace_bytes(R)
    ws = workspace.get("sweeps", ws_bytes, dev)
    check(L.fd_sweep_assemble(_p(raw), raw_cols, int(keep_cols), R, _p(desc_dev), n_desc, float(min_distance), _p(out),
                              _p(count), _p(ws), ws.numel(), _stream()), "fd_sweep_assemble")
    return out, count


def pillar_encode(voxels, num_points, coors4, n_dev, geom, layers, with_distance=False, out_dtype=torch.float32):
    L = _lib.load()
    voxels = _dev(voxels, "voxels", torch.float32)
    M, P, ndim = voxels.shape
    (w1, s1, b1) = layers[0]
    (w2, s2, b2) = layers[1] if len(layers) > 1 else (None, None, None)
    assert len(layers) in (1, 2)
    U = (w2 if w2 is not None else w1).shape[0]
    out = torch.zeros((M, U), dtype=out_dtype, device=voxels.device)
    check(L.fd_pillar_encode(_p(voxels), _p(num_points), _p(coors4), _p(n_dev), M, P, ndim, int(bool(with_distance)),
                             float(geom[0]), float(geom[1]), float(geom[2]), float(geom[3]), _p(w1), _p(s1), _p(b1), w1.shape[0],
                             _p(w2), _p(s2), _p(b2), (w2.shape[0] if w2 is not None else 0), _DT[out_dtype], _p(out), U, _stream()),
          "fd_pillar_encode")
    return out


def pillar_train_workspace_bytes(m, max_points):
    return int(_lib.load().fd_pillar_train_workspace_bytes(int(m), int(max_points)))


def _pillar_train_args(voxels, num_points, coors4, geom, w1, g1, b1, w2, g2, b2, with_distance):
    voxels = _dev(voxels, "voxels", torch.float32)
    M, P, ndim = voxels.shape
    for t, name in ((w1, "w1"), (g1, "gamma1"), (b1, "beta1"), (w2, "w2"), (g2, "gamma2"), (b2, "beta2")):
        _dev(t, name, torch.float32)
    return [_p(voxels), _p(_dev(num_points, "num_points", torch.int32)), _p(_dev(coors4, "coors4", torch.int32)), M, P, ndim,
            int(bool(with_distance)), float(geom[0]), float(geom[1]), float(geom[2]), float(geom[3])]


def pillar_train_forward(voxels, num_points, coors4, geom, w1, g1, b1, eps1, w2, g2, b2, eps2, with_distance=False, out=None,
                         workspace=None):
    L = _lib.load()
    args = _pillar_train_args(voxels, num_points, coors4, geom, w1, g1, b1, w2, g2, b2, with_distance)
    M, P = args[3], args[4]
    dev = voxels.device
    nbytes = L.fd_pillar_train_workspace_bytes(M, P)
    if workspace is None:
        workspace = torch.empty((max(int(nbytes), 256),), dtype=torch.uint8, device=dev)
    if out is None:
        out = torch.empty((M, w2.shape[0]), dtype=torch.float32, device=dev)
    stats = torch.empty((2 * w1.shape[0] + 2 * w2.shape[0],), dtype=torch.float32, device=dev)
    u1, u2 = w1.shape[0], w2.shape[0]
    mean1, var1, mean2, var2 = stats[:u1], stats[u1:2 * u1], stats[2 * u1:2 * u1 + u2], stats[2 * u1 + u2:]
    check(L.fd_pillar_train_forward(*args, _p(w1), _p(g1), _p(b1), u1, float(eps1), _p(w2), _p(g2), _p(b2), u2, float(eps2),
                                    _p(_dev(out, "out", torch.float32)), _p(mean1), _p(var1), _p(mean2), _p(var2), _p(workspace),
                                    workspace.numel(), _stream()), "fd_pillar_train_forward")
    return out, mean1, var1, mean2, var2, workspace


def pillar_train_backward(dout, voxels, num_points, coors4, geom, w1, g1, b1, w2, g2, b2, workspace, with_distance=False):
    L = _lib.load()
    args = _pillar_train_args(voxels, num_points, coors4, geom, w1, g1, b1, w2, g2, b2, with_distance)
    dout = _dev(dout, "dout", torch.float32)
    assert tuple(dout.shape) == (args[3], w2.shape[0]), (tuple(dout.shape), args[3])
    dw1, dw2 = torch.empty_like(w1), torch.empty_like(w2)
    dg1, db1, dg2, db2 = torch.empty_like(g1), torch.empty_like(b1), torch.empty_like(g2), torch.empty_like(b2)
    check(L.fd_pillar_train_backward(*args, _p(w1), _p(g1), _p(b1), w1.shape[0], _p(w2), _p(g2), _p(b2), w2.shape[0], _p(dout),
                                     _p(dw1), _p(dg1), _p(db1), _p(dw2), _p(dg2), _p(db2), _p(workspace), workspace.numel(), _stream()),
          "fd_pillar_train_backward")
    return dw1, dg1, db1, dw2, dg2, db2


def pillar_scatter_backward(dcanvas, coors4):
    L = _lib.load()
    if not (isinstance(dcanvas, torch.Tensor) and dcanvas.is_cuda and dcanvas.dtype == torch.float32):
        raise FutureDetHipError("pillar_scatter_backward: dcanvas must be a float32 tensor on the HIP device")
    coors4 = _dev(coors4, "coors4", torch.int32)
    n, c = coors4.shape[0], dcanvas.shape[1]
    feats = torch.empty((max(n, 1), c), dtype=torch.float32, device=dcanvas.device)[:n]
    sb, sc, sy, sx = dcanvas.stride()
    check(L.fd_dense_gather(_p(dcanvas), sb, sc, sy, sx, 1, _p(coors4), n, None, c, _p(feats), _stream()), "fd_dense_gather")
    return feats


def pillar_scatter(feats, coors4, n_dev, batch_size, ny, nx, out_dtype=None, channels_last=False, out=None, zero_first=True):
    L = _lib.load()
    feats = _dev(feats, "feats")
    M, C = feats.shape
    if out is None:
        out = torch.empty((batch_size, C, ny, nx), dtype=out_dtype or feats.dtype, device=feats.device,
                          memory_format=torch.channels_last if channels_last else torch.contiguous_format)
    sb, sc, sy, sx = out.stride()
    check(L.fd_pillar_scatter(_p(feats), C, feats.stride(0), _DT[feats.dtype], _p(coors4), _p(n_dev), M, batch_size, ny, nx,
                              _p(out), _DT[out.dtype], sb, sc, sy, sx, int(bool(zero_first)), _stream()), "fd_pillar_scatter")
    return out


def forecast_chains(centers, velocity, counts, time, reject_thresh):
    L = _lib.load()
    centers = _dev(centers, "centers", torch.float64)
    velocity = _dev(velocity, "velocity", torch.float64)
    T, n, _ = centers.shape
    dev = centers.device
    i32 = dict(dtype=torch.int32, device=dev)
    out = dict(fwd_idx=torch.zeros((n, T), **i32), fwd_ok=torch.zeros((n,), **i32), bwd_idx=torch.zeros((n, T), **i32),
               bwd_ok=torch.zeros((n,), **i32), match_idx=torch.zeros((T, n), **i32),
               cv_centers=torch.zeros((n, T, 3), dtype=torch.float64, device=dev), status=torch.zeros((1,), **i32))
    check(L.fd_forecast_chains(_p(centers), _p(velocity), _p(counts), _p(time), T, n, float(reject_thresh), _p(out["fwd_idx"]),
                               _p(out["fwd_ok"]), _p(out["bwd_idx"]), _p(out["bwd_ok"]), _p(out["match_idx"]), _p(out["cv_centers"]),
                               _p(out["status"]), _stream()), "fd_forecast_chains")
    return out


def det_to_global_boxes(box3d, cs_record=None, pose_record=None):
    L = _lib.load()
    box3d = _dev(box3d, "box3d", torch.float32)
    n = box3d.shape[0]
    assert box3d.shape[1] == 9, "box3d_lidar rows are (x,y,z,w,l,h,vx,vy,yaw)"
    dev = box3d.device
    center = torch.empty((n, 3), dtype=torch.float64, device=dev)
    quat = torch.empty((n, 4), dtype=torch.float64, device=dev)
    vel = torch.empty((n, 3), dtype=torch.float64, device=dev)
    size = torch.empty((n, 3), dtype=torch.float32, device=dev)

    def rec(r):
        if r is None:
            return None, None
        q, t = (ctypes.c_double * 4)(*[float(v) for v in r[0]]), (ctypes.c_double * 3)(*[float(v) for v in r[1]])
        return q, t

    cq, ct = rec(cs_record)
    pq, pt = rec(pose_record)
    check(L.fd_det_to_global_boxes(_p(box3d), n, cq, ct, pq, pt, _p(center), _p(quat), _p(vel), _p(size), _stream()), "fd_det_to_global_boxes")
    return center, quat, vel, size


def nearest_rows(library, queries):
    L = _lib.load()
    library, queries = _dev(library, "library", torch.float64), _dev(queries, "queries", torch.float64)
    assert library.shape[1] == queries.shape[1]
    idx = torch.zeros((max(queries.shape[0], 1),), dtype=torch.int32, device=queries.device)[: queries.shape[0]]
    check(L.fd_nearest_rows(_p(library), library.shape[0], _p(queries), queries.shape[0], library.shape[1], _p(idx), _stream()), "fd_nearest_rows")
    return idx


def forecast_groups(centers, match_thresh):
    L = _lib.load()
    centers = _dev(centers, "centers", torch.float64)
    n = centers.shape[0]
    ids = torch.zeros((max(n, 1),), dtype=torch.int32, device=centers.device)[:n]
    check(L.fd_forecast_groups(_p(centers), n, float(match_thresh), _p(ids), _stream()), "fd_forecast_groups")
    return ids


class ForecastOutputs(object):

    FIELDS = (("center", (-1, -2, 3), torch.float64), ("quat", (-1, -2, 4), torch.float64), ("velocity", (-1, -2, 3), torch.float64),
              ("size", (-1, -2, 3), torch.float32), ("fwd_idx", (-3, -1), torch.int32), ("fwd_ok", (-3,), torch.int32),
              ("bwd_idx", (-3, -1), torch.int32), ("bwd_ok", (-3,), torch.int32), ("match_idx", (-1, -3), torch.int32),
              ("cv_centers", (-3, -1, 3), torch.float64), ("status", (), torch.int32), ("traj_kind", (-4,), torch.int32),
              ("traj_src", (-4,), torch.int32), ("traj_first", (-4,), torch.int32), ("traj_group", (-4,), torch.int32), ("n_traj", (), torch.int32))

    def __init__(self, B, T, post, device):
        self.B, self.T, self.post = int(B), int(T), int(post)
        sub = {-1: self.T, -2: self.post, -3: self.post, -4: 3 * self.post}
        layout, off = [], 0
        for name, shape, dt in self.FIELDS:
            shape = (self.B,) + tuple(sub.get(d, d) for d in shape)
            nbytes = int(np.prod(shape)) * torch.empty((), dtype=dt).element_size()
            layout.append((name, shape, dt, off, nbytes))
            off = (off + nbytes + 15) & ~15
        self.layout = layout
        self.blob = torch.zeros((off,), dtype=torch.uint8, device=device)
        for name, shape, dt, o, nbytes in layout:
            setattr(self, name, self.blob[o:o + nbytes].view(dt).view(shape))
        self.c_struct = _lib.ForecastBuffers(**{name: getattr(self, name).data_ptr() for name, _, _ in self.FIELDS})

    def views_of(self, blob_host):
        a = blob_host.numpy() if isinstance(blob_host, torch.Tensor) else np.asarray(blob_host)
        npdt = {torch.float64: np.float64, torch.float32: np.float32, torch.int32: np.int32}
        return {name: a[o:o + nbytes].view(npdt[dt]).reshape(shape) for name, shape, dt, o, nbytes in self.layout}

    def host(self):
        return self.views_of(self.blob.cpu())


def forecast_from_detections(packed, counts, time, records=None, reject_thresh=2.0, match_thresh=0.25, out=None):
    L = _lib.load()
    packed = _dev(packed, "packed", torch.float32)
    counts = _dev(counts, "counts", torch.int32)
    time = _dev(time, "time", torch.float64)
    B, T, post, F = packed.shape
    assert tuple(counts.shape) == (B, T) and tuple(time.shape) == (B, T - 1)
    if records is not None:
        records = _dev(records, "records", torch.float64)
        assert tuple(records.shape) == (B, 14)
    if out is None:
        out = ForecastOutputs(B, T, post, packed.device)
    assert (out.B, out.T, out.post) == (B, T, post)
    check(L.fd_forecast_from_detections(_p(packed), _p(counts), B, T, post, F, _p(records), _p(time), float(reject_thresh), float(match_thresh),
                                        ctypes.byref(out.c_struct), _stream()), "fd_forecast_from_detections")
    return out
```

### futuredet_amd/lib.py

```python
import ctypes
import os

_HERE = os.path.dirname(os.path.abspath(__file__))
LIB_PATH = os.environ.get("FD_LIB_PATH") or os.path.join(_HERE, "libfuturedet_hip.so")
_lib = None

c_void_p = ctypes.c_void_p
c_int = ctypes.c_int
c_i64 = ctypes.c_int64
c_size_t = ctypes.c_size_t
c_float = ctypes.c_float


class MapView(ctypes.Structure):
    _fields_ = [("data", ctypes.c_void_p), ("group_stride", ctypes.c_int64), ("channel_stride", ctypes.c_int64), ("cell_stride", ctypes.c_int64),
                ("dtype", ctypes.c_int)]


ABI_VERSION = 8


class DecodeCfg(ctypes.Structure):
    _fields_ = [("H", c_int), ("W", c_int), ("out_size_factor", c_float), ("voxel_x", c_float), ("voxel_y", c_float),
                ("pc_x", c_float), ("pc_y", c_float), ("score_threshold", c_float), ("center_range", c_float * 6),
                ("nms_iou_threshold", c_float), ("nms_pre_max", c_int), ("nms_post_max", c_int), ("hm_channels", c_int),
                ("nms_kind", c_int), ("n_radius", c_int), ("circle_radius", c_float * 16)]


class IndexLevel(ctypes.Structure):
    _fields_ = [("D", ctypes.c_int32), ("H", ctypes.c_int32), ("W", ctypes.c_int32), ("ksize", ctypes.c_int32 * 3),
                ("stride", ctypes.c_int32 * 3), ("pad", ctypes.c_int32 * 3), ("words", c_void_p), ("prefix", c_void_p),
                ("coords", c_void_p), ("coords_rows", ctypes.c_int64)]


class ForecastBuffers(ctypes.Structure):
    _fields_ = [(n, c_void_p) for n in ("center", "quat", "velocity", "size", "fwd_idx", "fwd_ok", "bwd_idx", "bwd_ok", "match_idx", "cv_centers",
                                        "status", "traj_kind", "traj_src", "traj_first", "traj_group", "n_traj")]


class TargetsCfg(ctypes.Structure):
    _fields_ = [("H", c_int), ("W", c_int), ("T", c_int), ("n_max", c_int), ("max_objs", c_int), ("n_sets", c_int), ("n_tasks", c_int),
                ("task_classes", c_int * 16), ("radius_mult", c_int), ("min_radius", c_int), ("out_size_factor", c_float), ("voxel_x", c_float),
                ("voxel_y", c_float), ("pc_x", c_float), ("pc_y", c_float), ("gaussian_overlap", ctypes.c_double)]


SIGNATURES = {
    "fd_abi_version": (c_int, []),
    "fd_last_error": (ctypes.c_char_p, []),
    "fd_tuning_set": (c_int, [ctypes.c_char_p, c_int]),
    "fd_voxelize_workspace_bytes": (c_size_t, [c_i64, c_i64]),
    "fd_voxelize": (c_int, [c_void_p, c_i64, c_void_p, c_int, c_void_p, c_void_p, c_int, c_i64, c_int, c_void_p, c_void_p, c_int,
                            c_void_p, c_int, c_void_p, c_void_p, c_void_p, c_size_t, c_void_p]),
    "fd_index_num_cols": (c_i64, [c_int, c_int, c_int]),
    "fd_index_workspace_bytes": (c_size_t, [c_i64]),
    "fd_index_mark": (c_int, [c_void_p, c_void_p, c_i64, c_int, c_int, c_int, c_int, c_void_p, c_void_p]),
    "fd_index_downsample": (c_int, [c_void_p, c_int, c_int, c_int, c_int, c_void_p, c_void_p, c_void_p, c_void_p, c_void_p]),
    "fd_index_scan": (c_int, [c_void_p, c_i64, c_void_p, c_void_p, c_void_p, c_size_t, c_void_p]),
    "fd_index_coords": (c_int, [c_void_p, c_void_p, c_int, c_int, c_int, c_int, c_void_p, c_void_p]),
    "fd_index_lookup": (c_int, [c_void_p, c_void_p, c_int, c_int, c_int, c_int, c_void_p, c_void_p, c_i64, c_void_p, c_void_p]),
    "fd_rows_permute": (c_int, [c_void_p, c_int, c_void_p, c_void_p, c_i64, c_void_p, c_int, c_int, c_void_p]),
    "fd_rulebook": (c_int, [c_void_p, c_void_p, c_int, c_int, c_int, c_int, c_void_p, c_i64, c_void_p, c_i64, c_int, c_void_p, c_void_p,
                            c_void_p, c_void_p, c_void_p]),
    "fd_spconv_packed_weight_bytes": (c_size_t, [c_int, c_int, c_int, c_int]),
    "fd_spconv_pack_weight": (c_int, [c_void_p, c_int, c_int, c_int, c_int, c_void_p]),
    "fd_spconv_apply": (c_int, [c_void_p, c_i64, c_void_p, c_void_p, c_void_p, c_int, c_void_p, c_i64, c_void_p, c_int, c_int, c_i64,
                                c_void_p, c_i64, c_int, c_int, c_int, c_void_p, c_void_p]),
    "fd_spconv_num_ranges": (c_int, [c_i64, c_int, c_int, c_int]),
    "fd_spconv_wants_balanced_ranges": (c_int, [c_int, c_int, c_int]),
    "fd_spconv_ranges_workspace_bytes": (c_size_t, [c_i64]),
    "fd_spconv_ranges": (c_int, [c_void_p, c_i64, c_int, c_i64, c_void_p, c_int, c_void_p, c_void_p, c_size_t, c_void_p]),
    "fd_densify": (c_int, [c_void_p, c_int, c_int, c_void_p, c_void_p, c_int, c_int, c_int, c_int, c_void_p, c_int, c_i64,
                           c_i64, c_i64, c_i64, c_i64, c_void_p]),
    "fd_conv2d_packed_weight_bytes": (c_size_t, [c_int, c_int, c_int]),
    "fd_conv2d_pack_weight": (c_int, [c_void_p, c_int, c_int, c_int, c_void_p]),
    "fd_conv2d_nhwc_bf16": (c_int, [c_void_p, c_int, c_int, c_int, c_int, c_void_p, c_void_p, c_int, c_int, c_int, c_int, c_int,
                                    c_void_p, c_int, c_int, c_int, c_int, c_int, c_int, c_void_p]),
    "fd_conv2d_f32_packed_weight_bytes": (c_size_t, [c_int, c_int, c_int]),
    "fd_conv2d_f32_pack_weight": (c_int, [c_void_p, c_int, c_int, c_int, c_void_p]),
    "fd_conv2d_f32_num_tiles": (c_int, []),
    "fd_conv2d_nhwc_f32": (c_int, [c_void_p, c_int, c_int, c_int, c_int, c_void_p, c_void_p, c_int, c_int, c_int, c_int, c_int,
                                   c_void_p, c_int, c_int, c_int, c_int, c_int, c_int, c_int, c_void_p]),
    "fd_conv2d_shuffle_nhwc_f32": (c_int, [c_void_p, c_int, c_int, c_int, c_int, c_void_p, c_void_p, c_int, c_int, c_int, c_void_p, c_int, c_int, c_int,
                                           c_void_p]),
    "fd_conv2d_grouped_nhwc_f32": (c_int, [c_void_p, c_int, c_int, c_int, c_int, c_int, c_void_p, c_void_p, c_void_p, c_int, c_void_p, c_int, c_int,
                                           c_int, c_void_p]),
    "fd_conv2d_wino_f32_num_tiles": (c_int, []),
    "fd_conv2d_wino_f32_packed_weight_bytes": (c_size_t, [c_int, c_int]),
    "fd_conv2d_wino_f32_pack_weight": (c_int, [c_void_p, c_int, c_int, c_void_p]),
    "fd_conv2d_wino_nhwc_f32": (c_int, [c_void_p, c_int, c_int, c_int, c_int, c_void_p, c_void_p, c_int, c_int, c_void_p, c_int, c_int, c_int,
                                        c_void_p]),
    "fd_decode_workspace_bytes": (c_size_t, [c_int, ctypes.POINTER(DecodeCfg)]),
    "fd_centerpoint_decode": (c_int, [c_void_p, c_i64, c_void_p, c_i64, c_void_p, c_i64, c_void_p, c_i64, c_void_p, c_i64,
                                      c_int, ctypes.POINTER(DecodeCfg), c_void_p, c_void_p, c_void_p, c_void_p, c_void_p,
                                      c_size_t, c_void_p]),
    "fd_centerpoint_decode_maps": (c_int, [ctypes.POINTER(MapView)] * 5 + [c_int, ctypes.POINTER(DecodeCfg), c_void_p, c_void_p, c_void_p, c_void_p,
                                           c_void_p, c_size_t, c_void_p]),
    "fd_centerpoint_decode_packed": (c_int, [ctypes.POINTER(MapView)] * 6 + [c_int, c_int, ctypes.POINTER(DecodeCfg), c_int, c_void_p, c_void_p, c_void_p,
                                             c_void_p, c_void_p, c_void_p, c_void_p, c_void_p, c_void_p, c_void_p, c_size_t, c_void_p]),
    "fd_assemble_detections": (c_int, [c_void_p, c_void_p, c_void_p, c_void_p, ctypes.POINTER(MapView), c_int, c_int, c_int, c_void_p, c_void_p,
                                       c_void_p, c_void_p, c_void_p, c_void_p]),
    "fd_nms_workspace_bytes": (c_size_t, [c_int]),
    "fd_rotated_nms": (c_int, [c_void_p, c_int, c_float, c_void_p, c_void_p, c_void_p, c_size_t, c_void_p]),
    "fd_boxes_iou_bev": (c_int, [c_void_p, c_int, c_void_p, c_int, c_void_p, c_void_p]),
    "fd_pillar_encode": (c_int, [c_void_p, c_void_p, c_void_p, c_void_p, c_i64, c_int, c_int, c_int, c_float, c_float, c_float,
                                 c_float, c_void_p, c_void_p, c_void_p, c_int, c_void_p, c_void_p, c_void_p, c_int, c_int,
                                 c_void_p, c_int, c_void_p]),
    "fd_pillar_scatter": (c_int, [c_void_p, c_int, c_int, c_int, c_void_p, c_void_p, c_i64, c_int, c_int, c_int, c_void_p, c_int,
                                  c_i64, c_i64, c_i64, c_i64, c_int, c_void_p]),
    "fd_forecast_chains": (c_int, [c_void_p, c_void_p, c_void_p, c_void_p, c_int, c_int, ctypes.c_double, c_void_p, c_void_p,
                                   c_void_p, c_void_p, c_void_p, c_void_p, c_void_p, c_void_p]),
    "fd_det_to_global_boxes": (c_int, [c_void_p, c_int, c_void_p, c_void_p, c_void_p, c_void_p, c_void_p, c_void_p, c_void_p, c_void_p, c_void_p]),
    "fd_forecast_groups": (c_int, [c_void_p, c_int, ctypes.c_double, c_void_p, c_void_p]),
    "fd_forecast_from_detections": (c_int, [c_void_p, c_void_p, c_int, c_int, c_int, c_int, c_void_p, c_void_p, ctypes.c_double, ctypes.c_double,
                                            ctypes.POINTER(ForecastBuffers), c_void_p]),
    "fd_nearest_rows": (c_int, [c_void_p, c_int, c_void_p, c_int, c_int, c_void_p, c_void_p]),
    "fd_index_pyramid": (c_int, [c_void_p, c_void_p, c_i64, c_int, c_int, ctypes.POINTER(IndexLevel), c_void_p, c_void_p, c_size_t,
                                 c_void_p]),
    "fd_index_pyramid_coords": (c_int, [c_int, c_int, ctypes.POINTER(IndexLevel), c_void_p]),
    "fd_rows_place": (c_int, [c_void_p, c_void_p, c_int, c_int, c_int, c_int, c_void_p, c_void_p, c_i64, c_void_p, c_int, c_void_p,
                              c_int, c_int, c_void_p]),
    "fd_sweep_assemble_workspace_bytes": (c_size_t, [c_i64]),
    "fd_sweep_assemble": (c_int, [c_void_p, c_int, c_int, c_i64, c_void_p, c_int, c_float, c_void_p, c_void_p, c_void_p,
                                  c_size_t, c_void_p]),
    "fd_deform_adapt_packed_weight_bytes": (c_size_t, [c_int]),
    "fd_deform_adapt_pack_weight": (c_int, [c_void_p, c_void_p, c_int, c_void_p]),
    "fd_deform_adapt_nhwc": (c_int, [c_void_p, c_int, c_int, c_int, c_int, c_int, c_void_p, c_void_p, c_void_p, c_void_p, c_void_p, c_void_p]),
    "fd_deform_adapt_backward_workspace_bytes": (c_size_t, [c_int, c_int, c_int]),
    "fd_deform_adapt_backward": (c_int, [c_void_p, c_void_p, c_void_p, c_void_p, c_void_p, c_void_p, c_int, c_int, c_int, c_int, c_void_p, c_void_p,
                                         c_void_p, c_void_p, c_size_t, c_void_p]),
    "fd_deform_adapt_pack_weight_device": (c_int, [c_void_p, c_void_p, c_void_p, c_void_p]),
    "fd_spconv_wgrad_workspace_bytes": (c_size_t, [c_int, c_i64, c_int, c_int]),
    "fd_spconv_wgrad": (c_int, [c_void_p, c_i64, c_void_p, c_void_p, c_i64, c_int, c_i64, c_void_p, c_int, c_int, c_void_p, c_void_p, c_size_t,
                                c_void_p]),
    "fd_rulebook_transpose": (c_int, [c_void_p, c_i64, c_int, c_i64, c_void_p, c_i64, c_void_p, c_i64, c_void_p]),
    "fd_spconv_pack_weight_device": (c_int, [c_void_p, c_int, c_int, c_int, c_int, c_void_p, c_void_p]),
    "fd_dense_gather": (c_int, [c_void_p, c_i64, c_i64, c_i64, c_i64, c_int, c_void_p, c_i64, c_void_p, c_int, c_void_p, c_void_p]),
    "fd_pillar_train_workspace_bytes": (c_size_t, [c_i64, c_int]),
    "fd_pillar_train_forward": (c_int, [c_void_p, c_void_p, c_void_p, c_i64, c_int, c_int, c_int, c_float, c_float, c_float, c_float,
                                        c_void_p, c_void_p, c_void_p, c_int, c_float, c_void_p, c_void_p, c_void_p, c_int, c_float,
                                        c_void_p, c_void_p, c_void_p, c_void_p, c_void_p, c_void_p, c_size_t, c_void_p]),
    "fd_pillar_train_backward": (c_int, [c_void_p, c_void_p, c_void_p, c_i64, c_int, c_int, c_int, c_float, c_float, c_float, c_float,
                                         c_void_p, c_void_p, c_void_p, c_int, c_void_p, c_void_p, c_void_p, c_int, c_void_p,
                                         c_void_p, c_void_p, c_void_p, c_void_p, c_void_p, c_void_p, c_void_p, c_size_t, c_void_p]),
    "fd_targets_workspace_bytes": (c_size_t, [c_int, c_int, c_int, c_int]),
    "fd_assign_targets": (c_int, [c_void_p, c_void_p, c_void_p, c_void_p, c_int, ctypes.POINTER(TargetsCfg), c_void_p, c_void_p, c_void_p, c_void_p,
                                  c_void_p, c_void_p, c_void_p, c_void_p, c_size_t, c_void_p]),
}


class FutureDetHipError(RuntimeError):
    pass


def load():
    global _lib
    if _lib is None:
        if not os.path.isfile(LIB_PATH):
            raise FutureDetHipError(
                "libfuturedet_hip.so is not built (%s). Run `python -c 'import __graft_entry__ as g; g.build()'` "
                "or `python futuredet_amd/build.py`; there is no CPU fallback for this path." % LIB_PATH)
        L = ctypes.CDLL(LIB_PATH)
        for name, (res, args) in SIGNATURES.items():
            fn = getattr(L, name)
            fn.restype = res
            fn.argtypes = args
        if L.fd_abi_version() != ABI_VERSION:
            raise FutureDetHipError("%s reports ABI %d, these bindings are written for %d: rebuild it (python futuredet_amd/build.py --force)"
                                    % (LIB_PATH, L.fd_abi_version(), ABI_VERSION))
        _lib = L
    return _lib


def check(status, what):
    if status != 0:
        msg = load().fd_last_error()
        raise FutureDetHipError("%s failed (%d): %s" % (what, status, msg.decode() if msg else "?"))
```

### include/futuredet_hip.h

```cpp
#ifndef FUTUREDET_HIP_H
#define FUTUREDET_HIP_H

#include <stddef.h>
#include <stdint.h>

#ifdef __cplusplus
extern "C" {
#endif

#define FD_OK 0
#define FD_EINVAL (-1)
#define FD_EWORKSPACE (-2)
#define FD_ELAUNCH (-3)

typedef void *fd_stream_t;

int fd_abi_version(void);
const char *fd_last_error(void);
int fd_tuning_set(const char *name, int value);

size_t fd_voxelize_workspace_bytes(int64_t n_points, int64_t max_voxels);
int fd_voxelize(const float *points, int64_t n_points, const int32_t *n_points_dev, int ndim, const float *range6_host,
                const float *voxel_size3_host, int max_points, int64_t max_voxels, int batch_idx,
                float *out_voxels, float *out_mean, int mean_stride, int32_t *out_coors, int coor_cols,
                int32_t *out_num_points, int32_t *out_num_voxels, void *workspace, size_t workspace_bytes,
                fd_stream_t stream);

int64_t fd_index_num_cols(int B, int H, int W);
size_t fd_index_workspace_bytes(int64_t num_cols);
int fd_index_mark(const int32_t *coords , const int32_t *n_dev ,
                  int64_t n_max, int B, int D, int H, int W, uint64_t *words, fd_stream_t stream);
int fd_index_downsample(const uint64_t *in_words, int B, int D, int H, int W, const int *ksize3,
                        const int *stride3, const int *pad3, uint64_t *out_words, fd_stream_t stream);
int fd_index_scan(const uint64_t *words, int64_t num_cols, int32_t *prefix, int32_t *n_active_dev,
                  void *workspace, size_t workspace_bytes, fd_stream_t stream);
int fd_index_coords(const uint64_t *words, const int32_t *prefix, int B, int D, int H, int W,
                    int32_t *coords , fd_stream_t stream);
int fd_index_lookup(const uint64_t *words, const int32_t *prefix, int B, int D, int H, int W,
                    const int32_t *coords_in, const int32_t *n_dev, int64_t n_max, int32_t *row_of,
                    fd_stream_t stream);
int fd_rows_permute(const float *src, int c_src, const int32_t *row_of, const int32_t *n_dev, int64_t n_max,
                    void *dst, int c_dst, int dst_bf16, fd_stream_t stream);
int fd_rulebook(const uint64_t *in_words, const int32_t *in_prefix, int B, int Din, int Hin, int Win,
                const int32_t *out_coords, int64_t out_rows, const int32_t *n_out_dev, int64_t nbr_stride, int fill_tail, const int *ksize3,
                const int *stride3, const int *pad3, int32_t *nbr, fd_stream_t stream);

size_t fd_spconv_packed_weight_bytes(int K, int cin, int cout, int dtype);
int fd_spconv_pack_weight(const float *w_kio_host, int K, int cin, int cout, int dtype, void *wpacked_host);
int fd_spconv_apply(const void *in_feats, int64_t n_in, const void *wpacked, const float *bias, const void *residual,
                    int relu, const int32_t *nbr, int64_t nbr_stride, const int32_t *ranges ,
                    int n_ranges, int K, int64_t n_out, const int32_t *n_out_dev ,
                    int64_t n_expected ,
                    int cin, int cout, int dtype, void *out_feats, fd_stream_t stream);
int fd_spconv_num_ranges(int64_t n_out, int cin, int cout, int dtype);
int fd_spconv_wants_balanced_ranges(int cin, int cout, int dtype);
size_t fd_spconv_ranges_workspace_bytes(int64_t n_out);
int fd_spconv_ranges(const int32_t *nbr, int64_t nbr_stride, int K, int64_t n_out, const int32_t *n_out_dev, int n_ranges,
                     int32_t *ranges , void *workspace, size_t workspace_bytes, fd_stream_t stream);

int fd_densify(const void *feats, int c, int dtype, const uint64_t *words, const int32_t *prefix, int B, int D,
               int H, int W, void *out, int out_dtype, int64_t stride_b, int64_t stride_c, int64_t stride_y,
               int64_t stride_x, int64_t n_rows ,
               fd_stream_t stream);

size_t fd_conv2d_packed_weight_bytes(int cout, int cin, int ks);
int fd_conv2d_pack_weight(const float *w_oihw_host, int cout, int cin, int ks, void *wpacked_host);
int fd_conv2d_nhwc_bf16(const void *x, int B, int H, int W, int cin, const void *wpacked, const float *bias, int cout,
                        int ks, int stride, int pad, int relu, void *y, int cout_total, int co_off, int osy, int osx,
                        int ooy, int oox, fd_stream_t stream);
size_t fd_conv2d_f32_packed_weight_bytes(int cout, int cin, int ks);
int fd_conv2d_f32_pack_weight(const float *w_oihw_host, int cout, int cin, int ks, void *wpacked_host);
int fd_conv2d_f32_num_tiles(void);
int fd_conv2d_nhwc_f32(const float *x, int B, int H, int W, int cin, const void *wpacked, const float *bias, int cout, int ks,
                       int stride, int pad, int relu, float *y, int cout_total, int co_off, int osy, int osx, int ooy, int oox,
                       int tile , fd_stream_t stream);
int fd_conv2d_shuffle_nhwc_f32(const float *x, int B, int H, int W, int cin, const void *wpacked, const float *bias, int cout_sub, int k,
                               int relu, float *y, int cout_total, int co_off, int tile, fd_stream_t stream);
int fd_conv2d_grouped_nhwc_f32(const float *x, int B, int H, int W, int groups, int cin_g, const void *wpacked, const float *bias,
                               const int *counts_host, int relu, float *y, int cout_total, int co_off, int tile, fd_stream_t stream);
int fd_conv2d_wino_f32_num_tiles(void);
size_t fd_conv2d_wino_f32_packed_weight_bytes(int cout, int cin);
int fd_conv2d_wino_f32_pack_weight(const float *w_oihw_host, int cout, int cin, void *wpacked_host);
int fd_conv2d_wino_nhwc_f32(const float *x, int B, int H, int W, int cin, const void *wpacked, const float *bias, int cout, int relu,
                            float *y, int cout_total, int co_off, int tile , fd_stream_t stream);

typedef struct fd_decode_cfg {
    int H, W;
    float out_size_factor, voxel_x, voxel_y, pc_x, pc_y;
    float score_threshold;
    float center_range[6];
    float nms_iou_threshold;
    int nms_pre_max, nms_post_max;
    int hm_channels;
    int nms_kind;
    int n_radius;
    float circle_radius[16];
} fd_decode_cfg;

typedef struct fd_map_view {
    const void *data;
    int64_t group_stride, channel_stride, cell_stride;
    int dtype;
} fd_map_view;

size_t fd_decode_workspace_bytes(int G, const fd_decode_cfg *cfg);
int fd_centerpoint_decode_maps(const fd_map_view *hm, const fd_map_view *reg, const fd_map_view *height, const fd_map_view *dim,
                               const fd_map_view *rot, int G, const fd_decode_cfg *cfg_host, float *out_boxes7, float *out_scores,
                               int32_t *out_cell, int32_t *out_count, void *workspace, size_t workspace_bytes, fd_stream_t stream);
int fd_assemble_detections(const float *boxes7, const float *scores, const int32_t *cell, const int32_t *count, const fd_map_view *vel,
                           int B, int post_max, int S, const int32_t *step_group, const int32_t *step_vel_channel,
                           const int32_t *step_label, float *packed, int32_t *counts_out, fd_stream_t stream);
int fd_centerpoint_decode_packed(const fd_map_view *hm, const fd_map_view *reg, const fd_map_view *height, const fd_map_view *dim,
                                 const fd_map_view *rot, const fd_map_view *vel, int G, int B, const fd_decode_cfg *cfg_host, int S,
                                 const int32_t *step_group, const int32_t *step_vel_channel, const int32_t *step_label, float *out_boxes7,
                                 float *out_scores, int32_t *out_cell, int32_t *out_count, float *packed, int32_t *counts_out, void *workspace,
                                 size_t workspace_bytes, fd_stream_t stream);
int fd_centerpoint_decode(const float *hm, int64_t hm_gstride, const float *reg, int64_t reg_gstride,
                          const float *height, int64_t height_gstride, const float *dim, int64_t dim_gstride,
                          const float *rot, int64_t rot_gstride, int G, const fd_decode_cfg *cfg_host,
                          float *out_boxes7, float *out_scores, int32_t *out_cell, int32_t *out_count,
                          void *workspace, size_t workspace_bytes, fd_stream_t stream);

size_t fd_nms_workspace_bytes(int n);
int fd_rotated_nms(const float *boxes7, int n, float thresh, int64_t *keep, int32_t *out_count,
                   void *workspace, size_t workspace_bytes, fd_stream_t stream);
int fd_boxes_iou_bev(const float *a7, int na, const float *b7, int nb, float *out, fd_stream_t stream);

#define FD_SWEEP_HAS_TRANSFORM 1
#define FD_SWEEP_REMOVE_CLOSE 2
typedef struct fd_sweep_desc {
    double m[16];
    int64_t row_begin, row_end;
    float time;
    int32_t flags;
} fd_sweep_desc;
size_t fd_sweep_assemble_workspace_bytes(int64_t n_rows);
int fd_sweep_assemble(const float *raw, int raw_cols, int keep_cols, int64_t n_rows, const fd_sweep_desc *sweeps_dev,
                      int n_sweeps, float min_distance, float *out_points, int32_t *out_count, void *workspace,
                      size_t workspace_bytes, fd_stream_t stream);

int fd_pillar_encode(const float *voxels, const int32_t *num_points, const int32_t *coors4, const int32_t *n_dev,
                     int64_t m_max, int max_points, int ndim, int with_distance, float vx, float vy, float x_offset,
                     float y_offset, const float *w1, const float *scale1, const float *shift1, int units1,
                     const float *w2, const float *scale2, const float *shift2, int units2, int out_dtype, void *out,
                     int out_stride, fd_stream_t stream);

int fd_pillar_scatter(const void *feats, int c, int feat_stride, int dtype, const int32_t *coors4, const int32_t *n_dev,
                      int64_t m_max, int B, int H, int W, void *out, int out_dtype, int64_t stride_b, int64_t stride_c,
                      int64_t stride_y, int64_t stride_x, int zero_first, fd_stream_t stream);


int fd_forecast_chains(const double *centers, const double *velocity, const int32_t *counts, const double *time_dev, int T,
                       int n_max, double reject_thresh, int32_t *fwd_idx, int32_t *fwd_ok, int32_t *bwd_idx, int32_t *bwd_ok,
                       int32_t *match_idx, double *cv_centers, int32_t *status, fd_stream_t stream);

int fd_det_to_global_boxes(const float *box3d9, int n, const double *cs_rotation4_host, const double *cs_translation3_host,
                           const double *pose_rotation4_host, const double *pose_translation3_host, double *center,
                           double *quat, double *velocity, float *size, fd_stream_t stream);
int fd_forecast_groups(const double *centers3, int n, double match_thresh, int32_t *ids, fd_stream_t stream);

typedef struct fd_forecast_buffers {
    double *center, *quat, *velocity;
    float *size;
    int32_t *fwd_idx, *fwd_ok, *bwd_idx, *bwd_ok, *match_idx;
    double *cv_centers;
    int32_t *status;
    int32_t *traj_kind, *traj_src, *traj_first, *traj_group, *n_traj;
} fd_forecast_buffers;
int fd_forecast_from_detections(const float *packed, const int32_t *counts, int B, int T, int post, int row_floats,
                                const double *records_dev, const double *time_dev, double reject_thresh, double match_thresh,
                                const fd_forecast_buffers *out, fd_stream_t stream);

int fd_nearest_rows(const double *library, int n_library, const double *queries, int n_queries, int dim, int32_t *idx, fd_stream_t stream);

typedef struct fd_index_level {
    int32_t D, H, W;
    int32_t ksize[3], stride[3], pad[3];
    uint64_t *words;
    int32_t *prefix;
    int32_t *coords;
    int64_t coords_rows;
} fd_index_level;
int fd_index_pyramid(const int32_t *coords, const int32_t *n_dev, int64_t n_max_per_sample, int B, int n_levels,
                     const fd_index_level *levels_host, int32_t *counts_dev, void *workspace, size_t workspace_bytes,
                     fd_stream_t stream);
int fd_index_pyramid_coords(int B, int n_levels, const fd_index_level *levels_host, fd_stream_t stream);

int fd_rows_place(const uint64_t *words, const int32_t *prefix, int B, int D, int H, int W, const int32_t *coords_in,
                  const int32_t *n_dev, int64_t n_max, const float *src, int c_src, void *dst, int c_dst, int dst_bf16,
                  fd_stream_t stream);

size_t fd_deform_adapt_packed_weight_bytes(int bf16);
int fd_deform_adapt_pack_weight(const float *w_cls_oihw_host, const float *w_reg_oihw_host, int bf16, void *wpacked_host);
int fd_deform_adapt_nhwc(const void *x, int B, int H, int W, int C, int bf16, const float *off_w, const float *off_b, const float *offsets,
                         const void *wpacked, void *y, fd_stream_t stream);

size_t fd_deform_adapt_backward_workspace_bytes(int B, int H, int W);
int fd_deform_adapt_backward(const float *x, const float *offsets, const float *w_cls_oihw, const float *w_reg_oihw, const float *y, const float *dy,
                             int B, int H, int W, int C, float *dx, float *doffsets, float *dw, void *workspace, size_t workspace_bytes,
                             fd_stream_t stream);
int fd_deform_adapt_pack_weight_device(const float *w_cls_oihw, const float *w_reg_oihw, void *wpacked, fd_stream_t stream);

size_t fd_spconv_wgrad_workspace_bytes(int K, int64_t n_out, int cin, int cout);
int fd_spconv_wgrad(const float *in_feats, int64_t n_in, const float *dy, const int32_t *nbr, int64_t nbr_stride, int K, int64_t n_out,
                    const int32_t *n_out_dev, int cin, int cout, float *dw, void *workspace, size_t workspace_bytes, fd_stream_t stream);
int fd_rulebook_transpose(const int32_t *nbr, int64_t nbr_stride, int K, int64_t n_out, const int32_t *n_out_dev, int64_t n_in, int32_t *inv,
                          int64_t inv_stride, fd_stream_t stream);
int fd_spconv_pack_weight_device(const float *w_kio, int K, int cin, int cout, int mode, void *wpacked, fd_stream_t stream);
int fd_dense_gather(const float *dense, int64_t stride_b, int64_t stride_c, int64_t stride_y, int64_t stride_x, int D, const int32_t *coords,
                    int64_t n_rows, const int32_t *n_dev, int c, float *feats, fd_stream_t stream);

#define FD_TARGETS_MAX_TASKS 16
typedef struct fd_targets_cfg {
    int H, W;
    int T, n_max, max_objs;
    int n_sets;
    int n_tasks;
    int task_classes[FD_TARGETS_MAX_TASKS];
    int radius_mult;
    int min_radius;
    float out_size_factor, voxel_x, voxel_y, pc_x, pc_y;
    double gaussian_overlap;
} fd_targets_cfg;
size_t fd_targets_workspace_bytes(int B, int T, int maps_per_step, int max_objs);
int fd_assign_targets(const float *boxes, const int32_t *counts, const int32_t *classes, const int32_t *trajectory, int B,
                      const fd_targets_cfg *cfg, float *hm, int64_t *ind, uint8_t *mask, int64_t *cat, float *anno_box,
                      float *gt_boxes_and_cls, int32_t *status, void *workspace, size_t workspace_bytes, fd_stream_t stream);

size_t fd_pillar_train_workspace_bytes(int64_t m, int max_points);
int fd_pillar_train_forward(const float *voxels, const int32_t *num_points, const int32_t *coors4, int64_t m, int max_points, int ndim,
                            int with_distance, float vx, float vy, float x_offset, float y_offset, const float *w1, const float *gamma1,
                            const float *beta1, int units1, float eps1, const float *w2, const float *gamma2, const float *beta2, int units2,
                            float eps2, float *out, float *mean1, float *var1, float *mean2, float *var2, void *workspace,
                            size_t workspace_bytes, fd_stream_t stream);
int fd_pillar_train_backward(const float *voxels, const int32_t *num_points, const int32_t *coors4, int64_t m, int max_points, int ndim,
                             int with_distance, float vx, float vy, float x_offset, float y_offset, const float *w1, const float *gamma1,
                             const float *beta1, int units1, const float *w2, const float *gamma2, const float *beta2, int units2,
                             const float *dout, float *dw1, float *dgamma1, float *dbeta1, float *dw2, float *dgamma2, float *dbeta2,
                             void *workspace, size_t workspace_bytes, fd_stream_t stream);

#ifdef __cplusplus
}
#endif
#endif
```

Baseline: 282.1.

## Precompute per-chunk tap compaction plans for c32 submanifold spconv and reuse them

Adds a plan kernel that compacts the neighbour list and builds the per-wave item lists for each 128-row chunk once per rulebook. The c32 f32 kernel then loads these precomputed slots instead of running compaction and item building (with their barriers) in every conv that shares the rulebook. Plans are built on the side stream with the rulebooks and cached on the nbr tensor. It also changes how taps are split across the four waves for K=27, giving the centre tap its own split to rebalance work. The cost is extra memory and one additional plan kernel per rulebook, plus header checks in the kernel.

```diff
diff --git a/futuredet_amd/backbones.py b/futuredet_amd/backbones.py
--- a/futuredet_amd/backbones.py
+++ b/futuredet_amd/backbones.py
@@ -127,6 +127,8 @@
             wpk, bias, cin_p, cout_p = conv.packed_weight(dt, bn)
             assert x.shape[1] == cin_p, (x.shape, cin_p)
             nbr = rulebook(src, dst, conv)
+            if dt == torch.float32 and src is dst and cin_p == cout_p == 32:
+                hip_ops.plan_for(nbr, cin_p, cout_p)
             fn = lambda: hip_ops.spconv_apply(x, wpk, bias, nbr, dst.n, cout_p, residual=residual, relu=relu)
             if self.profile_hook is not None:
                 s = 4 if dt == torch.float32 else 2
@@ -160,6 +162,10 @@
                             r = hip_ops.ranges_for(nbr, cp, cp)
                             if r[0] is not None:
                                 made.append(r[0])
+                        if dt == torch.float32 and cp == 32:
+                            p = hip_ops.plan_for(nbr, cp, cp)
+                            if p is not None:
+                                made.append(p)
                 for t in made:
                     t.record_stream(main)
         x = feats0
diff --git a/futuredet_amd/csrc/fd_common.h b/futuredet_amd/csrc/fd_common.h
--- a/futuredet_amd/csrc/fd_common.h
+++ b/futuredet_amd/csrc/fd_common.h
@@ -29,7 +29,7 @@
 
 int spconv_f32_c32_dispatch(const float *in, const void *wp, const float *bias, const float *residual, int relu, const int *nbr,
                             int64_t nbr_stride, int K, int64_t n_in_bound, int n_out, const int *n_out_dev, int cin, int cout, float *out,
-                            const int *ranges, int n_ranges, hipStream_t stream);
+                            const int *ranges, int n_ranges, const void *plan, size_t plan_bytes, hipStream_t stream);
 
 __device__ __forceinline__ int device_count(int capacity, const int *count_dev) {
     if (!count_dev) return capacity;
diff --git a/futuredet_amd/csrc/fd_spconv.hip b/futuredet_amd/csrc/fd_spconv.hip
--- a/futuredet_amd/csrc/fd_spconv.hip
+++ b/futuredet_amd/csrc/fd_spconv.hip
@@ -314,9 +314,10 @@
     return FD_OK;
 }
 
-extern "C" int fd_spconv_apply(const void *in_feats, int64_t n_in, const void *wpacked, const float *bias, const void *residual, int relu,
-                               const int32_t *nbr, int64_t nbr_stride, const int32_t *ranges, int n_ranges, int K, int64_t n_out,
-                               const int32_t *n_out_dev, int64_t n_expected, int cin, int cout, int dtype, void *out_feats, fd_stream_t stream) {
+namespace {
+int spconv_apply_impl(const void *in_feats, int64_t n_in, const void *wpacked, const float *bias, const void *residual, int relu, const int32_t *nbr,
+                      int64_t nbr_stride, const int32_t *ranges, int n_ranges, int K, int64_t n_out, const int32_t *n_out_dev, int64_t n_expected, int cin,
+                      int cout, int dtype, void *out_feats, const void *plan, size_t plan_bytes, fd_stream_t stream) {
     FD_REQUIRE(K >= 1 && K <= kMaxTaps, "fd_spconv_apply: K must be in [1,27]");
     FD_REQUIRE(dtype == 0 || dtype == 1, "fd_spconv_apply: dtype must be 0 (f32) or 1 (bf16)");
     FD_REQUIRE(n_out >= 0 && n_out <= nbr_stride && n_out < (1ll << 31), "fd_spconv_apply: n_out out of range");
@@ -332,7 +333,7 @@
     if (dtype == 0 && !fd::tuning(fd::kTuneSpconvV1) && has_c32_layout(cin, cout, dtype) && fd::tuning(fd::kTuneSpconvC32) >= 0) {
         const void *w32 = (const char *)wpacked + (size_t)K * cin * cout * 4;
         if (fd::spconv_f32_c32_dispatch((const float *)in_feats, w32, bias, (const float *)residual, relu, nbr, nbr_stride, K, n_in, (int)n_out,
-                                        n_out_dev, cin, cout, (float *)out_feats, ranges, n_ranges, fd::as_stream(stream)))
+                                        n_out_dev, cin, cout, (float *)out_feats, ranges, n_ranges, plan, plan_bytes, fd::as_stream(stream)))
             return fd::check_launch("fd_spconv_apply(c32)");
     }
     if (dtype == 0 && !fd::tuning(fd::kTuneSpconvV1)) {
@@ -372,3 +373,20 @@
     }
     return fd::check_launch("fd_spconv_apply");
 }
+}
+
+extern "C" int fd_spconv_apply(const void *in_feats, int64_t n_in, const void *wpacked, const float *bias, const void *residual, int relu,
+                               const int32_t *nbr, int64_t nbr_stride, const int32_t *ranges, int n_ranges, int K, int64_t n_out,
+                               const int32_t *n_out_dev, int64_t n_expected, int cin, int cout, int dtype, void *out_feats, fd_stream_t stream) {
+    return spconv_apply_impl(in_feats, n_in, wpacked, bias, residual, relu, nbr, nbr_stride, ranges, n_ranges, K, n_out, n_out_dev, n_expected, cin, cout, dtype,
+                             out_feats, nullptr, 0, stream);
+}
+
+extern "C" int fd_spconv_apply_plan(const void *in_feats, int64_t n_in, const void *wpacked, const float *bias, const void *residual, int relu,
+                                    const int32_t *nbr, int64_t nbr_stride, const int32_t *ranges, int n_ranges, int K, int64_t n_out,
+                                    const int32_t *n_out_dev, int64_t n_expected, int cin, int cout, int dtype, void *out_feats, const void *plan,
+                                    size_t plan_bytes, fd_stream_t stream) {
+    FD_REQUIRE(plan == nullptr || plan_bytes >= 64, "fd_spconv_apply_plan: plan without its header");
+    return spconv_apply_impl(in_feats, n_in, wpacked, bias, residual, relu, nbr, nbr_stride, ranges, n_ranges, K, n_out, n_out_dev, n_expected, cin, cout, dtype,
+                             out_feats, plan, plan_bytes, stream);
+}
diff --git a/futuredet_amd/csrc/fd_spconv_c32.hip b/futuredet_amd/csrc/fd_spconv_c32.hip
--- a/futuredet_amd/csrc/fd_spconv_c32.hip
+++ b/futuredet_amd/csrc/fd_spconv_c32.hip
@@ -7,13 +7,71 @@
 typedef unsigned u32x4 __attribute__((ext_vector_type(4)));
 constexpr int TM = 128, COUT = 32, TS = 4, WR = 1;
 constexpr sk::Layout L = sk::layout(TM, COUT, TS, 32);
-static_assert(((sk::kMaxTaps + TS - 1) / TS) * (TM / WR / 32) <= L.item_slot, "item list slot");
-
-template <int CIN, int DEPTH>
+static_assert(sk::ceil_taps(sk::kMaxTaps, TS) * (TM / WR / 32) <= L.item_slot, "item list slot");
+
+#ifdef FD_C32_TRACE
+__device__ unsigned long long *g_c32_trace;
+constexpr unsigned kTraceWorkgroups = 4096;
+#define FD_C32_TW(i, v)                                                                                                   \
+    do {                                                                                                                  \
+        if (chunk == 0 && lane == 0 && g_c32_trace && blockIdx.x < kTraceWorkgroups)                                      \
+            g_c32_trace[((size_t)blockIdx.x * 4 + wave) * 8 + (i)] = (unsigned long long)(v);                             \
+    } while (0)
+#else
+#define FD_C32_TW(i, v)
+#endif
+
+struct PlanHeader { int magic, K, nbr_stride, n_out, n_ranges, rows_per_range, has_dev, chunk_slots; };
+constexpr int kPlanMagic = 0x43333270, kPlanHeaderBytes = 64;
+constexpr int kPlanNItems = L.pad;
+constexpr int kPlanSlotBytes = kPlanNItems + 16;
+static_assert(L.list == 0 && L.list < L.items && L.items < L.cnt && L.cnt < L.pad && L.item_slot == 32 && kPlanSlotBytes % 16 == 0 &&
+              sizeof(PlanHeader) <= kPlanHeaderBytes, "the plan slot mirrors the LDS layout");
+
+__device__ __forceinline__ const unsigned char *plan_slot(const unsigned char *plan, int chunk_slots, int chunk) {
+    return plan + kPlanHeaderBytes + ((size_t)blockIdx.x * chunk_slots + chunk) * kPlanSlotBytes;
+}
+
+__global__ void __launch_bounds__(256) c32_plan_kernel(const int *__restrict__ nbr, int64_t nbr_stride, int K, int n_out, const int *__restrict__ n_out_dev,
+                                                       int rows_per_range, int chunk_slots, unsigned char *__restrict__ plan) {
+    __shared__ __attribute__((aligned(16))) unsigned char smem[kPlanSlotBytes];
+    int *s_list = reinterpret_cast<int *>(smem + L.list);
+    unsigned short *s_items = reinterpret_cast<unsigned short *>(smem + L.items);
+    unsigned char *s_cnt = smem + L.cnt;
+    int *s_n = reinterpret_cast<int *>(smem + kPlanNItems);
+    const int tid = threadIdx.x, lane = tid & 63, wave = __builtin_amdgcn_readfirstlane(tid >> 6);
+    if (blockIdx.x == 0 && tid == 0) {
+        PlanHeader h{kPlanMagic, K, (int)nbr_stride, fd::device_count(n_out, n_out_dev), (int)gridDim.x, rows_per_range, n_out_dev ? 1 : 0, chunk_slots};
+        *reinterpret_cast<PlanHeader *>(plan) = h;
+    }
+    int r_begin, r_end, n_chunks, chunk_rows;
+    sk::resolve_range(n_out, n_out_dev, nullptr, rows_per_range, r_begin, r_end);
+    if (r_begin >= r_end) return;
+    sk::cut_chunks<TM>(r_begin, r_end, n_chunks, chunk_rows);
+    if (n_chunks > chunk_slots) return;
+    for (int chunk = 0; chunk < n_chunks; ++chunk) {
+        int row0, n_rows;
+        if (!sk::chunk_span(r_begin, r_end, chunk_rows, chunk, row0, n_rows)) break;
+        int pre[sk::kSliceRegs<TM>];
+        sk::fetch_slice<TM>(pre, nbr, nbr_stride, K, row0);
+        sk::stage_list<TM>(pre, s_list, K, n_rows);
+        __syncthreads();
+        sk::compact_taps<TM, WR>(s_list, s_cnt, K);
+        __syncthreads();
+        const int n_items = sk::build_items<TS, 32>(s_cnt, s_items + wave * L.item_slot, K, wave, 0);
+        if (lane == 0) s_n[wave] = n_items;
+        __syncthreads();
+        int4 *dst = reinterpret_cast<int4 *>(const_cast<unsigned char *>(plan_slot(plan, chunk_slots, chunk)));
+        for (int t = tid; t < kPlanSlotBytes / 16; t += 256) dst[t] = reinterpret_cast<const int4 *>(smem)[t];
+        __syncthreads();
+    }
+}
+
+template <int CIN, int DEPTH, bool PLAN>
 __global__ void __launch_bounds__(256) spconv_f32_c32(const float *__restrict__ in, const float4 *__restrict__ wp, const float *__restrict__ bias,
                                                       const float *__restrict__ residual, int relu, const int *__restrict__ nbr, int64_t nbr_stride,
                                                       int K, int n_out, const int *__restrict__ n_out_dev, float *__restrict__ out, unsigned in_bytes,
-                                                      const int *__restrict__ ranges, int rows_per_range) {
+                                                      const int *__restrict__ ranges, int rows_per_range, const unsigned char *__restrict__ plan, int plan_chunk_slots) {
     constexpr int NCH = CIN / 8;
     constexpr int kPad = sk::pad_entry(TM);
     extern __shared__ __attribute__((aligned(16))) unsigned char smem[];
@@ -28,8 +86,31 @@
     sk::resolve_range(n_out, n_out_dev, ranges, rows_per_range, r_begin, r_end);
     if (r_begin >= r_end) return;
     sk::cut_chunks<TM>(r_begin, r_end, n_chunks, chunk_rows);
+    bool planned = false;
+    int chunk_slots = 0;
+    if constexpr (PLAN) {
+        const PlanHeader *h = reinterpret_cast<const PlanHeader *>(plan);
+        chunk_slots = plan_chunk_slots;
+        planned = ranges == nullptr && h->chunk_slots == chunk_slots && h->magic == kPlanMagic && h->K == K && h->nbr_stride == (int)nbr_stride && h->n_out == fd::device_count(n_out, n_out_dev) &&
+                  h->n_ranges == (int)gridDim.x && h->rows_per_range == rows_per_range && h->has_dev == (n_out_dev ? 1 : 0) && n_chunks <= chunk_slots;
+    }
     int pre[sk::kSliceRegs<TM>];
-    sk::fetch_slice<TM>(pre, nbr, nbr_stride, K, r_begin);
+    int pre_item = 0, pre_n = 0;
+    auto fetch = [&](int chunk, int row0) {
+        if (PLAN && planned) {
+            const unsigned char *slot = plan_slot(plan, chunk_slots, chunk);
+#pragma unroll
+            for (int i = 0; i < sk::kSliceRegs<TM>; ++i) {
+                const int t = tid + i * 256;
+                pre[i] = reinterpret_cast<const int *>(slot + L.list)[t < K * TM ? t : K * TM - 1];
+            }
+            pre_item = (int)reinterpret_cast<const unsigned short *>(slot + L.items)[wave * L.item_slot + (lane & 31)];
+            pre_n = reinterpret_cast<const int *>(slot + kPlanNItems)[wave];
+        } else {
+            sk::fetch_slice<TM>(pre, nbr, nbr_stride, K, row0);
+        }
+    };
+    fetch(0, r_begin);
 
     const int ln = lane & 31, lh = lane >> 5;
     const int ts = wave, wr = 0;
@@ -40,12 +121,27 @@
     for (int chunk = 0; chunk < n_chunks; ++chunk) {
         int row0, n_rows;
         if (!sk::chunk_span(r_begin, r_end, chunk_rows, chunk, row0, n_rows)) break;
-        sk::stage_chunk<TM, COUT, TS, 32>(pre, s_list, s_pad, s_acc, bias, residual, K, row0, n_rows);
-        __syncthreads();
-        sk::compact_taps<TM, WR>(s_list, s_cnt, K);
-        __syncthreads();
-        if (chunk + 1 < n_chunks) sk::fetch_slice<TM>(pre, nbr, nbr_stride, K, row0 + chunk_rows);
-        const int n_items = sk::build_items<TS, 32>(s_cnt, items, K, ts, wr);
+        int n_items;
+        if (PLAN && planned) {
+#pragma unroll
+            for (int i = 0; i < sk::kSliceRegs<TM>; ++i) {
+                const int t = tid + i * 256;
+                if (t < K * TM) s_list[t] = pre[i];
+            }
+            if (lane < L.item_slot) items[lane] = (unsigned short)pre_item;
+            n_items = __builtin_amdgcn_readfirstlane(pre_n < L.item_slot ? pre_n : L.item_slot);
+            sk::init_acc<TM, COUT, TS>(s_acc, bias, residual, row0, n_rows);
+            if (tid < 32) s_pad[tid] = kPad;
+            __syncthreads();
+            if (chunk + 1 < n_chunks) fetch(chunk + 1, row0 + chunk_rows);
+        } else {
+            sk::stage_chunk<TM, COUT, TS, 32>(pre, s_list, s_pad, s_acc, bias, residual, K, row0, n_rows);
+            __syncthreads();
+            sk::compact_taps<TM, WR>(s_list, s_cnt, K);
+            __syncthreads();
+            if (chunk + 1 < n_chunks) fetch(chunk + 1, row0 + chunk_rows);
+            n_items = sk::build_items<TS, 32>(s_cnt, items, K, ts, wr);
+        }
 
         int k_r[DEPTH], row_r[DEPTH];
         u32x4 a_r[DEPTH][NCH];
@@ -74,6 +170,11 @@
         stage_a1(DEPTH - 1, stage_a0(DEPTH - 1), k_s, e_s);
         code_s = stage_a0(DEPTH);
         if (n_items > 0) load_b(k_r[0]);
+        FD_C32_TW(0, n_items);
+        FD_C32_TW(1, __builtin_amdgcn_s_getreg(4 | (31 << 11)));
+        FD_C32_TW(2, __builtin_amdgcn_s_getreg(20 | (31 << 11)));
+        FD_C32_TW(6, n_chunks);
+        FD_C32_TW(3, __builtin_readcyclecounter());
 
         for (int i0 = 0; i0 < n_items; i0 += DEPTH) {
 #pragma unroll
@@ -117,36 +218,86 @@
                 __builtin_amdgcn_sched_barrier(0);
             }
         }
-        __syncthreads();
+        FD_C32_TW(4, __builtin_readcyclecounter());
+        __syncthreads();
+        FD_C32_TW(5, __builtin_readcyclecounter());
         sk::epilogue<TM, COUT, TS>(s_acc, bias, residual, relu, out, row0, n_rows);
         __syncthreads();
     }
+}
+
+inline void plan_geometry(int n_out, bool device_count, int &n_ranges, int &rows_per, int &chunk_slots) {
+    sk::equal_rows_split(n_out, TM, device_count, n_ranges, rows_per);
+    chunk_slots = (rows_per + TM - 1) / TM;
+}
+inline size_t plan_bytes_for(int n_ranges, int chunk_slots) { return (size_t)kPlanHeaderBytes + (size_t)n_ranges * chunk_slots * kPlanSlotBytes; }
+
+template <int CIN, int DEPTH, bool PLAN>
+int launch_c32_kernel(const float *in, const void *wp, const float *bias, const float *residual, int relu, const int *nbr, int64_t nbr_stride, int K,
+                      int n_out, const int *n_out_dev, float *out, unsigned in_bytes, const int *ranges, int n_ranges, int rows_per,
+                      const unsigned char *plan, int chunk_slots, hipStream_t stream) {
+    static std::atomic<uint64_t> lds_set{0};
+    if (!fd::ensure_dynamic_lds(reinterpret_cast<const void *>(spconv_f32_c32<CIN, DEPTH, PLAN>), (size_t)L.bytes, lds_set)) return 0;
+    hipLaunchKernelGGL((spconv_f32_c32<CIN, DEPTH, PLAN>), dim3((unsigned)n_ranges), dim3(256), (size_t)L.bytes, stream, in, (const float4 *)wp, bias, residual, relu,
+                       nbr, nbr_stride, K, n_out, n_out_dev, out, in_bytes, ranges, rows_per, plan, chunk_slots);
+    return 1;
 }
 
 template <int CIN, int DEPTH>
 int launch_c32(const float *in, const void *wp, const float *bias, const float *residual, int relu, const int *nbr, int64_t nbr_stride, int K,
-               int n_out, const int *n_out_dev, float *out, unsigned in_bytes, const int *ranges, int n_ranges, hipStream_t stream) {
-    int rows_per = 0;
-    if (!ranges) sk::equal_rows_split(n_out, TM, n_out_dev != nullptr, n_ranges, rows_per);
-    static std::atomic<uint64_t> lds_set{0};
-    if (!fd::ensure_dynamic_lds(reinterpret_cast<const void *>(spconv_f32_c32<CIN, DEPTH>), (size_t)L.bytes, lds_set)) return 0;
-    hipLaunchKernelGGL((spconv_f32_c32<CIN, DEPTH>), dim3((unsigned)n_ranges), dim3(256), (size_t)L.bytes, stream, in, (const float4 *)wp, bias, residual, relu,
-                       nbr, nbr_stride, K, n_out, n_out_dev, out, in_bytes, ranges, rows_per);
-    return 1;
-}
-
+               int n_out, const int *n_out_dev, float *out, unsigned in_bytes, const int *ranges, int n_ranges, const void *plan, size_t plan_bytes,
+               hipStream_t stream) {
+    int rows_per = 0, chunk_slots = 0;
+    if (!ranges) plan_geometry(n_out, n_out_dev != nullptr, n_ranges, rows_per, chunk_slots);
+    if (plan && !ranges && nbr_stride < (1ll << 31) && plan_bytes >= plan_bytes_for(n_ranges, chunk_slots))
+        return launch_c32_kernel<CIN, DEPTH, true>(in, wp, bias, residual, relu, nbr, nbr_stride, K, n_out, n_out_dev, out, in_bytes, ranges, n_ranges, rows_per,
+                                                   (const unsigned char *)plan, chunk_slots, stream);
+    return launch_c32_kernel<CIN, DEPTH, false>(in, wp, bias, residual, relu, nbr, nbr_stride, K, n_out, n_out_dev, out, in_bytes, ranges, n_ranges, rows_per,
+                                                nullptr, 0, stream);
+}
+
+}
+
+#ifdef FD_C32_TRACE
+extern "C" int fd_debug_set_c32_trace(void *p) { return hipMemcpyToSymbol(HIP_SYMBOL(g_c32_trace), &p, sizeof(p)) == hipSuccess ? 0 : -1; }
+#endif
+
+extern "C" int fd_spconv_tap_split(int K, int n_splits, int tap) {
+    if (K < 1 || K > sk::kMaxTaps || tap < 0 || tap >= K) return -1;
+    return n_splits == 4 ? sk::tap_split<4>(tap, K) : n_splits == 2 ? sk::tap_split<2>(tap, K) : n_splits == 1 ? 0 : -1;
+}
+
+extern "C" size_t fd_spconv_plan_bytes(int64_t n_out, int K, int cin, int cout, int dtype, int n_ranges, int device_count) {
+    if (dtype != 0 || cin != 32 || cout != 32 || K < 1 || K > sk::kMaxTaps || n_out <= 0 || n_out >= (1ll << 31) || n_ranges < 0) return 0;
+    int rows_per = 0, chunk_slots = 0;
+    plan_geometry((int)n_out, device_count != 0, n_ranges, rows_per, chunk_slots);
+    return plan_bytes_for(n_ranges, chunk_slots);
+}
+
+extern "C" int fd_spconv_plan_build(const int32_t *nbr, int64_t nbr_stride, int K, int64_t n_out, const int32_t *n_out_dev, int cin, int cout, int dtype,
+                                    int n_ranges, void *plan, size_t plan_bytes, fd_stream_t stream) {
+    FD_REQUIRE(nbr && plan, "fd_spconv_plan_build: null argument");
+    FD_REQUIRE(n_out >= 1 && n_out <= nbr_stride && nbr_stride < (1ll << 31), "fd_spconv_plan_build: bad sizes");
+    const size_t need = fd_spconv_plan_bytes(n_out, K, cin, cout, dtype, n_ranges, n_out_dev != nullptr);
+    FD_REQUIRE(need > 0, "fd_spconv_plan_build: this layer shape takes no plan (fd_spconv_plan_bytes)");
+    FD_REQUIRE(plan_bytes >= need, "fd_spconv_plan_build: plan buffer too small");
+    int rows_per = 0, chunk_slots = 0;
+    plan_geometry((int)n_out, n_out_dev != nullptr, n_ranges, rows_per, chunk_slots);
+    hipLaunchKernelGGL(c32_plan_kernel, dim3((unsigned)n_ranges), dim3(256), 0, fd::as_stream(stream), nbr, nbr_stride, K, (int)n_out, n_out_dev, rows_per,
+                       chunk_slots, (unsigned char *)plan);
+    return fd::check_launch("fd_spconv_plan_build");
 }
 
 namespace fd {
 int spconv_f32_c32_dispatch(const float *in, const void *wp, const float *bias, const float *residual, int relu, const int *nbr, int64_t nbr_stride,
                             int K, int64_t n_in_bound, int n_out, const int *n_out_dev, int cin, int cout, float *out, const int *ranges,
-                            int n_ranges, hipStream_t stream) {
+                            int n_ranges, const void *plan, size_t plan_bytes, hipStream_t stream) {
     if (cout != 32 || cin != 32) return 0;
     if (!sk::entries_fit(n_in_bound, cin)) return 0;
     const unsigned in_bytes = (unsigned)(n_in_bound * cin * 4);
     const int depth = fd::tuning(fd::kTuneV2Depth);
-    if (depth == 2) return launch_c32<32, 2>(in, wp, bias, residual, relu, nbr, nbr_stride, K, n_out, n_out_dev, out, in_bytes, ranges, n_ranges, stream);
-    if (depth == 4) return launch_c32<32, 4>(in, wp, bias, residual, relu, nbr, nbr_stride, K, n_out, n_out_dev, out, in_bytes, ranges, n_ranges, stream);
-    return launch_c32<32, 3>(in, wp, bias, residual, relu, nbr, nbr_stride, K, n_out, n_out_dev, out, in_bytes, ranges, n_ranges, stream);
-}
-}
+    if (depth == 2) return launch_c32<32, 2>(in, wp, bias, residual, relu, nbr, nbr_stride, K, n_out, n_out_dev, out, in_bytes, ranges, n_ranges, plan, plan_bytes, stream);
+    if (depth == 4) return launch_c32<32, 4>(in, wp, bias, residual, relu, nbr, nbr_stride, K, n_out, n_out_dev, out, in_bytes, ranges, n_ranges, plan, plan_bytes, stream);
+    return launch_c32<32, 3>(in, wp, bias, residual, relu, nbr, nbr_stride, K, n_out, n_out_dev, out, in_bytes, ranges, n_ranges, plan, plan_bytes, stream);
+}
+}
diff --git a/futuredet_amd/csrc/fd_spconv_chunk.h b/futuredet_amd/csrc/fd_spconv_chunk.h
--- a/futuredet_amd/csrc/fd_spconv_chunk.h
+++ b/futuredet_amd/csrc/fd_spconv_chunk.h
@@ -142,19 +142,23 @@
     }
 }
 
+template <int TM>
+__device__ __forceinline__ void stage_list(const int (&pre)[kSliceRegs<TM>], int *s_list, int K, int n_rows) {
+    const int tid = threadIdx.x;
+    static_assert(256 % TM == 0, "a thread stages the same local row in every pass");
+    const bool in_chunk = tid % TM < n_rows;
+#pragma unroll
+    for (int i = 0; i < kSliceRegs<TM>; ++i) {
+        const int t = tid + i * 256;
+        if (t < K * TM) s_list[t] = in_chunk ? pre[i] : -1;
+    }
+}
 template <int TM, int COUT, int TS, int ITEM>
 __device__ __forceinline__ void stage_chunk(const int (&pre)[kSliceRegs<TM>], int *s_list, int *s_pad, float *s_acc, const float *bias,
                                             const float *residual, int K, int row0, int n_rows) {
-    const int tid = threadIdx.x;
-    static_assert(256 % TM == 0, "a thread stages the same local row in every pass");
-    const bool in_chunk = tid % TM < n_rows;
-#pragma unroll
-    for (int i = 0; i < kSliceRegs<TM>; ++i) {
-        const int t = tid + i * 256;
-        if (t < K * TM) s_list[t] = in_chunk ? pre[i] : -1;
-    }
+    stage_list<TM>(pre, s_list, K, n_rows);
     init_acc<TM, COUT, TS>(s_acc, bias, residual, row0, n_rows);
-    if (tid < ITEM) s_pad[tid] = pad_entry(TM);
+    if (threadIdx.x < ITEM) s_pad[threadIdx.x] = pad_entry(TM);
 }
 
 template <int TM, int WR>
@@ -190,10 +194,37 @@
     }
 }
 
+constexpr int kCentreTap27 = 13;
+template <int TS>
+__host__ __device__ constexpr int tap_split(int k, int K) {
+#ifndef FD_TAPS_MOD
+    if (TS == 4 && K == 27) return k == kCentreTap27 ? 3 : (k == 15 ? 1 : (k & 3));
+#endif
+    return k % TS;
+}
+template <int TS>
+constexpr int taps_in_split(int ts, int K) {
+    int n = 0;
+    for (int k = 0; k < K; ++k) n += tap_split<TS>(k, K) == ts ? 1 : 0;
+    return n;
+}
+constexpr int ceil_taps(int K, int ts_count) { return (K + ts_count - 1) / ts_count; }
+template <int TS>
+constexpr bool tap_splits_fit() {
+    for (int K = 1; K <= kMaxTaps; ++K)
+        for (int ts = 0; ts < TS; ++ts)
+            if (taps_in_split<TS>(ts, K) > ceil_taps(K, TS)) return false;
+    return true;
+}
+static_assert(tap_splits_fit<1>() && tap_splits_fit<2>() && tap_splits_fit<4>(), "a split holds at most ceil(K / TS) taps");
+#ifndef FD_TAPS_MOD
+static_assert(taps_in_split<4>(3, 27) == 6 && tap_split<4>(kCentreTap27, 27) == 3, "the centre tap belongs to the split of six");
+#endif
+
 template <int TS, int ITEM>
 __device__ __forceinline__ int build_items(const unsigned char *s_cnt, unsigned short *items, int K, int ts, int wr) {
     const int lane = threadIdx.x & 63;
-    const int ng = (lane < K && (lane % TS) == ts) ? ((int)s_cnt[lane * 4 + wr] + ITEM - 1) / ITEM : 0;
+    const int ng = (lane < K && tap_split<TS>(lane, K) == ts) ? ((int)s_cnt[lane * 4 + wr] + ITEM - 1) / ITEM : 0;
     int inc = ng;
 #pragma unroll
     for (int off = 1; off < 64; off <<= 1) {
diff --git a/futuredet_amd/hip_ops.py b/futuredet_amd/hip_ops.py
--- a/futuredet_amd/hip_ops.py
+++ b/futuredet_amd/hip_ops.py
@@ -283,6 +283,28 @@
     return nbr.ranges
 
 
+def plan_for(nbr, cin, cout, n_ranges=None):
+    L = _lib.load()
+    n_out = getattr(nbr, "n_out", None)
+    if not n_out:
+        return None
+    K, nstride = nbr.shape
+    n_dev = getattr(nbr, "n_dev", None)
+    if n_ranges is None:
+        n_ranges = int(L.fd_spconv_num_ranges(getattr(nbr, "n_expected", 0) or n_out, cin, cout, 0))
+    cached = getattr(nbr, "plan", None)
+    if cached is not None and cached[1] == n_ranges:
+        return cached[0]
+    nbytes = int(L.fd_spconv_plan_bytes(n_out, K, cin, cout, 0, n_ranges, int(n_dev is not None)))
+    if nbytes <= 0:
+        return None
+    plan = torch.empty((nbytes,), dtype=torch.uint8, device=nbr.device)
+    check(L.fd_spconv_plan_build(_p(_dev(nbr, "nbr", torch.int32)), nstride, K, n_out, _p(n_dev), cin, cout, 0, n_ranges, _p(plan), nbytes, _stream()),
+          "fd_spconv_plan_build")
+    nbr.plan = (plan, n_ranges)
+    return plan
+
+
 def rows_permute(src, row_of, c_dst, dtype=torch.float32, n_rows=None, n_dev=None):
     L = _lib.load()
     src = _dev(src, "src", torch.float32)
@@ -394,7 +416,7 @@
     return feats
 
 
-def spconv_apply(feats, wpacked, bias, nbr, n_out, cout, residual=None, relu=False, out=None, balanced=None):
+def spconv_apply(feats, wpacked, bias, nbr, n_out, cout, residual=None, relu=False, out=None, balanced=None, plan=None):
     L = _lib.load()
     feats = _dev(feats, "feats")
     dt = _DT[feats.dtype]
@@ -416,6 +438,15 @@
             ranges, n_ranges = ranges_for(nbr, cin, cout)
         else:
             n_ranges = int(L.fd_spconv_num_ranges(n_expected or n_out, cin, cout, 0))
+    if plan is None:
+        cached = getattr(nbr, "plan", None)
+        plan = cached[0] if cached else None
+    if plan is not None and plan is not False and dt == 0:
+        check(L.fd_spconv_apply_plan(_p(feats), feats.shape[0], _p(_dev(wpacked, "wpacked")), _p(bias), _p(residual), int(bool(relu)),
+                                     _p(_dev(nbr, "nbr", torch.int32)), nstride, _p(ranges), n_ranges, K, n_out, _p(n_dev), int(n_expected or 0),
+                                     cin, cout, dt, _p(out), _p(_dev(plan, "plan", torch.uint8)), plan.numel(), _stream()),
+              "fd_spconv_apply_plan")
+        return out
     check(L.fd_spconv_apply(_p(feats), feats.shape[0], _p(_dev(wpacked, "wpacked")), _p(bias), _p(residual), int(bool(relu)),
                             _p(_dev(nbr, "nbr", torch.int32)), nstride, _p(ranges), n_ranges, K, n_out, _p(n_dev), int(n_expected or 0),
                             cin, cout, dt, _p(out), _stream()),
diff --git a/futuredet_amd/lib.py b/futuredet_amd/lib.py
--- a/futuredet_amd/lib.py
+++ b/futuredet_amd/lib.py
@@ -67,6 +67,11 @@
                                 c_void_p, c_i64, c_int, c_int, c_int, c_void_p, c_void_p]),
     "fd_spconv_num_ranges": (c_int, [c_i64, c_int, c_int, c_int]),
     "fd_spconv_wants_balanced_ranges": (c_int, [c_int, c_int, c_int]),
+    "fd_spconv_tap_split": (c_int, [c_int, c_int, c_int]),
+    "fd_spconv_plan_bytes": (c_size_t, [c_i64, c_int, c_int, c_int, c_int, c_int, c_int]),
+    "fd_spconv_plan_build": (c_int, [c_void_p, c_i64, c_int, c_i64, c_void_p, c_int, c_int, c_int, c_int, c_void_p, c_size_t, c_void_p]),
+    "fd_spconv_apply_plan": (c_int, [c_void_p, c_i64, c_void_p, c_void_p, c_void_p, c_int, c_void_p, c_i64, c_void_p, c_int, c_int, c_i64,
+                                     c_void_p, c_i64, c_int, c_int, c_int, c_void_p, c_void_p, c_size_t, c_void_p]),
     "fd_spconv_ranges_workspace_bytes": (c_size_t, [c_i64]),
     "fd_spconv_ranges": (c_int, [c_void_p, c_i64, c_int, c_i64, c_void_p, c_int, c_void_p, c_void_p, c_size_t, c_void_p]),
     "fd_densify": (c_int, [c_void_p, c_int, c_int, c_void_p, c_void_p, c_int, c_int, c_int, c_int, c_void_p, c_int, c_i64,
diff --git a/include/futuredet_hip.h b/include/futuredet_hip.h
--- a/include/futuredet_hip.h
+++ b/include/futuredet_hip.h
@@ -54,6 +54,14 @@
                     int cin, int cout, int dtype, void *out_feats, fd_stream_t stream);
 int fd_spconv_num_ranges(int64_t n_out, int cin, int cout, int dtype);
 int fd_spconv_wants_balanced_ranges(int cin, int cout, int dtype);
+int fd_spconv_tap_split(int K, int n_splits, int tap);
+size_t fd_spconv_plan_bytes(int64_t n_out, int K, int cin, int cout, int dtype, int n_ranges, int device_count );
+int fd_spconv_plan_build(const int32_t *nbr, int64_t nbr_stride, int K, int64_t n_out, const int32_t *n_out_dev, int cin, int cout,
+                         int dtype, int n_ranges, void *plan, size_t plan_bytes, fd_stream_t stream);
+int fd_spconv_apply_plan(const void *in_feats, int64_t n_in, const void *wpacked, const float *bias, const void *residual,
+                         int relu, const int32_t *nbr, int64_t nbr_stride, const int32_t *ranges, int n_ranges, int K, int64_t n_out,
+                         const int32_t *n_out_dev, int64_t n_expected, int cin, int cout, int dtype, void *out_feats,
+                         const void *plan, size_t plan_bytes, fd_stream_t stream);
 size_t fd_spconv_ranges_workspace_bytes(int64_t n_out);
 int fd_spconv_ranges(const int32_t *nbr, int64_t nbr_stride, int K, int64_t n_out, const int32_t *n_out_dev, int n_ranges,
                      int32_t *ranges , void *workspace, size_t workspace_bytes, fd_stream_t stream);
```

Result: no change. 284.0 (median of 6 runs) (+0.7%).
